# dominikbuenger/torch_nfft

Hardware: AMD Instinct MI355X
Metric: Mpoints/s (adjoint+forward, 3-D N=256 m=4) (higher is better)
Workload: dtype f32

## Files before the change

torch_nfft_amd/csrc/colfft.hip:

```cpp
#include <type_traits>

#include "common.h"
#include "kernels.h"

namespace nfft {

namespace {

constexpr int kFftThreads = 256;

struct ColGeom {
    int M, logM, N, H;
    int Mh;
    int SR;
    int KC;
    int KS;
    int NB;
    int NBm;
    int two_d;
    int NC, logNC;
    int TG;
    float param;
};

__device__ __forceinline__ float phi_hat_inv_f(int k, float param) { return expf((float)k * (float)k * param); }

__device__ __forceinline__ float2 cmul(float2 a, float2 b)
{
    return make_float2(a.x * b.x - a.y * b.y, a.x * b.y + a.y * b.x);
}

__device__ __forceinline__ void column_tile_of_block(const int tg, int &tile, int &row, int64_t &plane)
{
    const unsigned gx = gridDim.x, gy = gridDim.y;
    unsigned long long id = blockIdx.x + (unsigned long long)gx * (blockIdx.y + (unsigned long long)gy * blockIdx.z);
    if (tg > 1) {
        const unsigned long long total = (unsigned long long)gx * gy * gridDim.z;
        const unsigned span = 8u * (unsigned)tg;
        const unsigned long long base = id - id % span;
        if (base + span <= total) {
            const unsigned r = (unsigned)(id - base);
            id = base + (unsigned long long)(r & 7u) * (unsigned)tg + (r >> 3);
        }
    }
    tile = (int)(id % gx);
    const unsigned long long q = id / gx;
    row = (int)(q % gy);
    plane = (int64_t)(q / gy);
}

constexpr double kPiD = 3.14159265358979323846264338327950288;
constexpr double taylor_sin(double x)
{
    double term = x, sum = x;
    for (int k = 1; k <= 16; ++k) {
        term *= -x * x / (double)((2 * k) * (2 * k + 1));
        sum += term;
    }
    return sum;
}
constexpr double taylor_cos(double x)
{
    double term = 1.0, sum = 1.0;
    for (int k = 1; k <= 16; ++k) {
        term *= -x * x / (double)((2 * k - 1) * (2 * k));
        sum += term;
    }
    return sum;
}
struct TwPair { float x, y; };
template <int M>
struct TwTable { TwPair v[M / 2]; };
template <int M>
constexpr TwTable<M> make_tw_table()
{
    TwTable<M> t{};
    for (int j = 0; j < M / 2; ++j) {
        const bool upper = 4 * j > M;
        const double a = 2.0 * kPiD * (double)(upper ? M / 2 - j : j) / (double)M;
        const double c = taylor_cos(a), sn = taylor_sin(a);
        t.v[j] = TwPair{(float)(upper ? -c : c), (float)-sn};
    }
    return t;
}
template <int M>
__device__ const TwTable<M> kTwTable = make_tw_table<M>();

template <int M>
const float2 *tw_symbol()
{
    void *ptr = nullptr;
    if (hipGetSymbolAddress(&ptr, HIP_SYMBOL(kTwTable<M>)) != hipSuccess) return nullptr;
    return (const float2 *)ptr;
}
const float2 *twiddle_table(int M)
{
    static std::atomic<const float2 *> cache[kMaxDevices][7];
    const int dev = current_device();
    int slot = 0;
    while ((16 << slot) < M) ++slot;
    if (slot > 6 || (16 << slot) != M) return nullptr;
    if (dev < kMaxDevices) {
        const float2 *p = cache[dev][slot].load(std::memory_order_acquire);
        if (p) return p;
    }
    const float2 *p = nullptr;
    switch (M) {
    case 16: p = tw_symbol<16>(); break;
    case 32: p = tw_symbol<32>(); break;
    case 64: p = tw_symbol<64>(); break;
    case 128: p = tw_symbol<128>(); break;
    case 256: p = tw_symbol<256>(); break;
    case 512: p = tw_symbol<512>(); break;
    case 1024: p = tw_symbol<1024>(); break;
    }
    if (p && dev < kMaxDevices) cache[dev][slot].store(p, std::memory_order_release);
    return p;
}

__device__ __forceinline__ float2 cadd(float2 a, float2 b) { return make_float2(a.x + b.x, a.y + b.y); }
__device__ __forceinline__ float2 csub(float2 a, float2 b) { return make_float2(a.x - b.x, a.y - b.y); }
template <bool INV>
__device__ __forceinline__ float2 rot90(float2 a)
{
    return INV ? make_float2(-a.y, a.x) : make_float2(a.y, -a.x);
}

template <bool INV>
__device__ __forceinline__ void dft4(float2 &x0, float2 &x1, float2 &x2, float2 &x3)
{
    const float2 a0 = cadd(x0, x2), a1 = csub(x0, x2), a2 = cadd(x1, x3), a3 = rot90<INV>(csub(x1, x3));
    x0 = cadd(a0, a2);
    x1 = cadd(a1, a3);
    x2 = csub(a0, a2);
    x3 = csub(a1, a3);
}

template <bool INV>
__device__ __forceinline__ void dft8(float2 (&x)[8])
{
    dft4<INV>(x[0], x[2], x[4], x[6]);
    dft4<INV>(x[1], x[3], x[5], x[7]);
    constexpr float r = 0.70710678118654752440f;
    const float2 o0 = x[1];
    const float2 o1 = INV ? make_float2((x[3].x - x[3].y) * r, (x[3].x + x[3].y) * r)
                          : make_float2((x[3].x + x[3].y) * r, (x[3].y - x[3].x) * r);
    const float2 o2 = rot90<INV>(x[5]);
    const float2 o3 = INV ? make_float2((-x[7].x - x[7].y) * r, (x[7].x - x[7].y) * r)
                          : make_float2((x[7].y - x[7].x) * r, (-x[7].x - x[7].y) * r);
    const float2 e0 = x[0], e1 = x[2], e2 = x[4], e3 = x[6];
    x[0] = cadd(e0, o0); x[4] = csub(e0, o0);
    x[1] = cadd(e1, o1); x[5] = csub(e1, o1);
    x[2] = cadd(e2, o2); x[6] = csub(e2, o2);
    x[3] = cadd(e3, o3); x[7] = csub(e3, o3);
}

template <bool INV>
__device__ __forceinline__ float2 twiddle_at(const float2 *ltw, int e, int M)
{
    e &= M - 1;
    float2 w = ltw[e & (M / 2 - 1)];
    if (e >= M / 2) w = make_float2(-w.x, -w.y);
    if (INV) w.y = -w.y;
    return w;
}

template <bool INV, int R>
__device__ __forceinline__ void fft_stage(float2 *buf, const float2 *ltw, const ColGeom &cg, int tid, int logL)
{
    constexpr int logR = R == 8 ? 3 : 2;
    const int logLs = logL - logR, Ls = 1 << logLs;
    const int tstep = cg.M >> logL;
    const int total = (cg.M >> logR) << cg.logNC;
    __syncthreads();
    for (int idx = tid; idx < total; idx += kFftThreads) {
        const int col = idx & (cg.NC - 1);
        const int t = idx >> cg.logNC;
        const int j = t & (Ls - 1);
        const int row0 = ((t >> logLs) << logL) + j;
        float2 *p0 = buf + (row0 << cg.logNC) + col;
        const int stride = Ls << cg.logNC;
        float2 x[R];
#pragma unroll
        for (int q = 0; q < R; ++q) x[q] = p0[q * stride];
        if (R == 8) {
            dft8<INV>(reinterpret_cast<float2(&)[8]>(x));
        } else {
            dft4<INV>(x[0], x[1], x[2], x[3]);
        }
        p0[0] = x[0];
        if (logLs == 0) {
#pragma unroll
            for (int q = 1; q < R; ++q) p0[q * stride] = x[q];
        } else {
#pragma unroll
            for (int q = 1; q < R; ++q) p0[q * stride] = cmul(x[q], twiddle_at<INV>(ltw, j * q * tstep, cg.M));
        }
    }
}

template <bool INV>
__device__ __forceinline__ void lds_fft(float2 *buf, const float2 *ltw, const ColGeom &cg, int tid)
{
    switch (cg.logM) {
    case 4: fft_stage<INV, 4>(buf, ltw, cg, tid, 4); fft_stage<INV, 4>(buf, ltw, cg, tid, 2); break;
    case 5: fft_stage<INV, 8>(buf, ltw, cg, tid, 5); fft_stage<INV, 4>(buf, ltw, cg, tid, 2); break;
    case 6: fft_stage<INV, 8>(buf, ltw, cg, tid, 6); fft_stage<INV, 8>(buf, ltw, cg, tid, 3); break;
    case 7: fft_stage<INV, 8>(buf, ltw, cg, tid, 7); fft_stage<INV, 4>(buf, ltw, cg, tid, 4);
            fft_stage<INV, 4>(buf, ltw, cg, tid, 2); break;
    case 8: fft_stage<INV, 8>(buf, ltw, cg, tid, 8); fft_stage<INV, 8>(buf, ltw, cg, tid, 5);
            fft_stage<INV, 4>(buf, ltw, cg, tid, 2); break;
    case 9: fft_stage<INV, 8>(buf, ltw, cg, tid, 9); fft_stage<INV, 8>(buf, ltw, cg, tid, 6);
            fft_stage<INV, 8>(buf, ltw, cg, tid, 3); break;
    default: fft_stage<INV, 8>(buf, ltw, cg, tid, 10); fft_stage<INV, 8>(buf, ltw, cg, tid, 7);
             fft_stage<INV, 4>(buf, ltw, cg, tid, 4); fft_stage<INV, 4>(buf, ltw, cg, tid, 2); break;
    }
    __syncthreads();
}

__device__ __forceinline__ int brev_row(int k, int logM)
{
    int pos = 0, lg = logM;
    auto digit = [&](int lr) { lg -= lr; pos += (k & ((1 << lr) - 1)) << lg; k >>= lr; };
    switch (logM) {
    case 4: digit(2); digit(2); break;
    case 5: digit(3); digit(2); break;
    case 6: digit(3); digit(3); break;
    case 7: digit(3); digit(2); digit(2); break;
    case 8: digit(3); digit(3); digit(2); break;
    case 9: digit(3); digit(3); digit(3); break;
    default: digit(3); digit(3); digit(2); digit(2); break;
    }
    return pos;
}

template <int UN, typename LoadF, typename StoreF>
__device__ __forceinline__ void batched_fill(int total, int tid, LoadF load, StoreF store)
{
    for (int base = tid; base < total; base += kFftThreads * UN) {
        float2 v[UN];
#pragma unroll
        for (int r = 0; r < UN; ++r) {
            const int idx = base + r * kFftThreads;
            v[r] = idx < total ? load(idx) : make_float2(0.f, 0.f);
        }
#pragma unroll
        for (int r = 0; r < UN; ++r) {
            const int idx = base + r * kFftThreads;
            if (idx < total) store(idx, v[r]);
        }
    }
}

__device__ __forceinline__ void stage_twiddles(float2 *ltw, const float2 *__restrict__ tw, int M, int tid)
{
    for (int j = tid; j < M / 2; j += kFftThreads) ltw[j] = tw[j];
}

template <int LOGM, int LOGNC>
__global__ void __launch_bounds__(kFftThreads)
adj_axis1_kernel(ColGeom cg_in, const float2 *__restrict__ tw, const float2 *__restrict__ S, float2 *__restrict__ T)
{
    ColGeom cg = cg_in;
    if constexpr (LOGM > 0) {
        cg.M = 1 << LOGM;
        cg.logM = LOGM;
        cg.NC = 1 << LOGNC;
        cg.logNC = LOGNC;
    }
    extern __shared__ float2 smem[];
    float2 *ltw = smem;
    float2 *buf = smem + cg.M / 2;
    const int tid = threadIdx.x;
    int tile_x, u0;
    int64_t plane;
    column_tile_of_block(cg.TG, tile_x, u0, plane);
    const int c0 = tile_x << cg.logNC;
    if (c0 >= cg.KC) return;
    stage_twiddles(ltw, tw, cg.M, tid);
    const float2 *src = S + ((plane * cg.M + u0) * cg.M) * cg.SR;
    batched_fill<16>(cg.M << cg.logNC, tid,
                     [&](int idx) {
                         const int col = idx & (cg.NC - 1), u1 = idx >> cg.logNC;
                         const int k2 = c0 + col;
                         return k2 < cg.KC ? src[(int64_t)u1 * cg.SR + k2] : make_float2(0.f, 0.f);
                     },
                     [&](int idx, float2 v) { buf[idx] = v; });
    lds_fft<false>(buf, ltw, cg, tid);
    float2 *dst = T + ((plane * cg.M + u0) * cg.NB) * cg.KS;
    for (int idx = tid; idx < (cg.NB << cg.logNC); idx += kFftThreads) {
        const int col = idx & (cg.NC - 1), j1 = idx >> cg.logNC;
        const int k2 = c0 + col;
        if (k2 < cg.KC) {
            const int k1 = (j1 - cg.H) & (cg.M - 1);
            dst[(int64_t)j1 * cg.KS + k2] = buf[(brev_row(k1, cg.logM) << cg.logNC) + col];
        }
    }
}

__device__ __forceinline__ void apply_mult(const void *__restrict__ mult, int kind, int64_t f, float &re, float &im)
{
    if (kind == 1) {
        const float w = ((const float *)mult)[f];
        re *= w;
        im *= w;
    } else if (kind == 2) {
        const float2 w = ((const float2 *)mult)[f];
        const float r2 = re * w.x - im * w.y;
        im = re * w.y + im * w.x;
        re = r2;
    }
}

template <int LOGM, int LOGNC, bool XCOMPLEX, bool REAL_OUT>
__global__ void __launch_bounds__(kFftThreads)
adj_axis0_kernel(ColGeom cg_in, const float2 *__restrict__ tw, const float2 *__restrict__ T, int64_t C, int64_t col0,
                 void *__restrict__ yv, const void *__restrict__ mult, int mult_kind)
{
    ColGeom cg = cg_in;
    if constexpr (LOGM > 0) {
        cg.M = 1 << LOGM;
        cg.logM = LOGM;
        cg.NC = 1 << LOGNC;
        cg.logNC = LOGNC;
    }
    extern __shared__ float2 smem[];
    float2 *ltw = smem;
    float2 *buf = smem + cg.M / 2;
    float2 *buf2 = buf + (cg.M << cg.logNC);
    const int tid = threadIdx.x;
    int tile_x, j1;
    int64_t col_local;
    column_tile_of_block(cg.TG, tile_x, j1, col_local);
    const int c0 = tile_x << cg.logNC;
    if (c0 >= cg.KC) return;
    stage_twiddles(ltw, tw, cg.M, tid);
    const int64_t plane = XCOMPLEX ? col_local * 2 : col_local;
    const int64_t pstride = (int64_t)cg.M * cg.NBm * cg.KS;
    const float2 *src = T + plane * pstride + (int64_t)j1 * cg.KS;
    for (int part = 0; part < (XCOMPLEX ? 2 : 1); ++part) {
        float2 *const dstbuf = part ? buf2 : buf;
        const float2 *const srcp = src + part * pstride;
        batched_fill<16>(cg.M << cg.logNC, tid,
                         [&](int idx) {
                             const int col = idx & (cg.NC - 1), u0 = idx >> cg.logNC;
                             const int k2 = c0 + col;
                             return k2 < cg.KC ? srcp[(int64_t)u0 * cg.NBm * cg.KS + k2] : make_float2(0.f, 0.f);
                         },
                         [&](int idx, float2 v) { dstbuf[idx] = v; });
    }
    lds_fft<false>(buf, ltw, cg, tid);
    if (XCOMPLEX) lds_fft<false>(buf2, ltw, cg, tid);

    const int64_t colg = col0 + col_local;
    const int64_t b = colg / C, c = colg - b * C;
    const int H = cg.H, N = cg.N;
    const int k1 = cg.two_d ? 0 : j1 - H;
    const float f1 = cg.two_d ? 1.0f : phi_hat_inv_f(abs(k1), cg.param);
    const int64_t NN = cg.two_d ? (int64_t)N * N : (int64_t)N * N * N;
    for (int idx = tid; idx < (cg.NB << cg.logNC); idx += kFftThreads) {
        const int col = idx & (cg.NC - 1), j0 = idx >> cg.logNC;
        const int k2 = c0 + col;
        if (k2 >= cg.KC) continue;
        const int k0 = j0 - H;
        const int row = (brev_row(k0 & (cg.M - 1), cg.logM) << cg.logNC) + col;
        const float2 fr = buf[row];
        float2 fi = make_float2(0.f, 0.f);
        if (XCOMPLEX) fi = buf2[row];
        const float fac = phi_hat_inv_f(abs(k0), cg.param) * f1 * phi_hat_inv_f(k2, cg.param);
        if (k0 < H && k1 < H && k2 < H) {
            float re = (fr.x + fi.y) * fac, im = (-fr.y + fi.x) * fac;
            const int64_t f = cg.two_d ? (int64_t)(k0 + H) * N + (k2 + H) : ((int64_t)(k0 + H) * N + (k1 + H)) * N + (k2 + H);
            apply_mult(mult, mult_kind, f, re, im);
            const int64_t o = (b * NN + f) * C + c;
            if (REAL_OUT) ((float *)yv)[o] = re;
            else ((float2 *)yv)[o] = make_float2(re, im);
        }
        if (k2 >= 1 && k0 > -H && k1 > -H) {
            float re = (fr.x - fi.y) * fac, im = (fr.y + fi.x) * fac;
            const int64_t f = cg.two_d ? (int64_t)(H - k0) * N + (H - k2) : ((int64_t)(H - k0) * N + (H - k1)) * N + (H - k2);
            apply_mult(mult, mult_kind, f, re, im);
            const int64_t o = (b * NN + f) * C + c;
            if (REAL_OUT) ((float *)yv)[o] = re;
            else ((float2 *)yv)[o] = make_float2(re, im);
        }
    }
}

template <bool XCOMPLEX>
__device__ __forceinline__ float2 band_value(const void *__restrict__ xhat, int64_t b, int64_t c, int64_t C, int N,
                                             int H, int k0, int k1, int k2, const bool two_d = false)
{
    if (k0 < -H || k0 >= H || (!two_d && (k1 < -H || k1 >= H)) || k2 < -H || k2 >= H) return make_float2(0.f, 0.f);
    const int64_t idx = two_d ? ((b * N + (k0 + H)) * N + (k2 + H)) * C + c
                              : (((b * N + (k0 + H)) * N + (k1 + H)) * N + (k2 + H)) * C + c;
    if (XCOMPLEX) return ((const float2 *)xhat)[idx];
    return make_float2(((const float *)xhat)[idx], 0.f);
}

template <int LOGM, int LOGNC, bool XCOMPLEX>
__global__ void __launch_bounds__(kFftThreads)
fwd_axis0_kernel(ColGeom cg_in, const float2 *__restrict__ tw, const void *__restrict__ xhat, int64_t C, int ppc,
                 int64_t plane0, float2 *__restrict__ T)
{
    ColGeom cg = cg_in;
    if constexpr (LOGM > 0) {
        cg.M = 1 << LOGM;
        cg.logM = LOGM;
        cg.NC = 1 << LOGNC;
        cg.logNC = LOGNC;
    }
    extern __shared__ float2 smem[];
    float2 *ltw = smem;
    float2 *buf = smem + cg.M / 2;
    const int tid = threadIdx.x;
    int tile_x, j1;
    int64_t pl;
    column_tile_of_block(cg.TG, tile_x, j1, pl);
    const int c0 = tile_x << cg.logNC;
    if (c0 >= cg.KC) return;
    stage_twiddles(ltw, tw, cg.M, tid);
    for (int idx = tid; idx < (cg.M << cg.logNC); idx += kFftThreads) buf[idx] = make_float2(0.f, 0.f);
    __syncthreads();
    const int64_t plane = plane0 + pl;
    const int64_t colg = plane / ppc;
    const int part = (int)(plane - colg * ppc);
    const int64_t b = colg / C, c = colg - b * C;
    const int H = cg.H;
    const int k1 = cg.two_d ? 0 : j1 - H;
    const float f1 = cg.two_d ? 1.0f : phi_hat_inv_f(abs(k1), cg.param);
    batched_fill<8>(cg.NB << cg.logNC, tid,
                    [&](int idx) {
                        const int col = idx & (cg.NC - 1), j0 = idx >> cg.logNC;
                        const int k2 = c0 + col;
                        if (k2 >= cg.KC) return make_float2(0.f, 0.f);
                        const int k0 = j0 - H;
                        const float2 ap = band_value<XCOMPLEX>(xhat, b, c, C, cg.N, H, k0, k1, k2, cg.two_d != 0);
                        const float2 am = band_value<XCOMPLEX>(xhat, b, c, C, cg.N, H, -k0, -k1, -k2, cg.two_d != 0);
                        const float fac = 0.5f * phi_hat_inv_f(abs(k0), cg.param) * f1 * phi_hat_inv_f(k2, cg.param);
                        if (part == 0) return make_float2((am.x + ap.x) * fac, (am.y - ap.y) * fac);
                        return make_float2((am.y + ap.y) * fac, -(am.x - ap.x) * fac);
                    },
                    [&](int idx, float2 v) {
                        const int col = idx & (cg.NC - 1), j0 = idx >> cg.logNC;
                        if (c0 + col < cg.KC) buf[(((j0 - H) & (cg.M - 1)) << cg.logNC) + col] = v;
                    });
    lds_fft<true>(buf, ltw, cg, tid);
    float2 *dst = T + pl * ((int64_t)cg.M * cg.NBm * cg.KS) + (int64_t)j1 * cg.KS;
    for (int idx = tid; idx < (cg.M << cg.logNC); idx += kFftThreads) {
        const int col = idx & (cg.NC - 1), u0 = idx >> cg.logNC;
        const int k2 = c0 + col;
        if (k2 < cg.KC) dst[(int64_t)u0 * cg.NBm * cg.KS + k2] = buf[(brev_row(u0, cg.logM) << cg.logNC) + col];
    }
}

template <int LOGM, int LOGNC>
__global__ void __launch_bounds__(kFftThreads)
fwd_axis1_kernel(ColGeom cg_in, const float2 *__restrict__ tw, const float2 *__restrict__ T, float2 *__restrict__ S)
{
    ColGeom cg = cg_in;
    if constexpr (LOGM > 0) {
        cg.M = 1 << LOGM;
        cg.logM = LOGM;
        cg.NC = 1 << LOGNC;
        cg.logNC = LOGNC;
    }
    extern __shared__ float2 smem[];
    float2 *ltw = smem;
    float2 *buf = smem + cg.M / 2;
    const int tid = threadIdx.x;
    int tile_x, u0;
    int64_t plane;
    column_tile_of_block(cg.TG, tile_x, u0, plane);
    const int c0 = tile_x << cg.logNC;
    if (c0 >= (cg.SR == cg.KS ? cg.KC : cg.Mh)) return;
    float2 *dst = S + ((plane * cg.M + u0) * cg.M) * cg.SR;
    const int width = cg.SR == cg.KS ? cg.KC : cg.Mh;
    if (c0 >= cg.KC) {
        for (int idx = tid; idx < (cg.M << cg.logNC); idx += kFftThreads) {
            const int col = idx & (cg.NC - 1), u1 = idx >> cg.logNC;
            if (c0 + col < width) dst[(int64_t)u1 * cg.SR + c0 + col] = make_float2(0.f, 0.f);
        }
        return;
    }
    stage_twiddles(ltw, tw, cg.M, tid);
    for (int idx = tid; idx < (cg.M << cg.logNC); idx += kFftThreads) buf[idx] = make_float2(0.f, 0.f);
    __syncthreads();
    const float2 *src = T + ((plane * cg.M + u0) * cg.NB) * cg.KS;
    batched_fill<16>(cg.NB << cg.logNC, tid,
                     [&](int idx) {
                         const int col = idx & (cg.NC - 1), j1 = idx >> cg.logNC;
                         const int k2 = c0 + col;
                         return k2 < cg.KC ? src[(int64_t)j1 * cg.KS + k2] : make_float2(0.f, 0.f);
                     },
                     [&](int idx, float2 v) {
                         const int col = idx & (cg.NC - 1), j1 = idx >> cg.logNC;
                         if (c0 + col < cg.KC) buf[(((j1 - cg.H) & (cg.M - 1)) << cg.logNC) + col] = v;
                     });
    lds_fft<true>(buf, ltw, cg, tid);
    for (int idx = tid; idx < (cg.M << cg.logNC); idx += kFftThreads) {
        const int col = idx & (cg.NC - 1), u1 = idx >> cg.logNC;
        const int k2 = c0 + col;
        if (k2 < width) {
            dst[(int64_t)u1 * cg.SR + k2] =
                k2 < cg.KC ? buf[(brev_row(u1, cg.logM) << cg.logNC) + col] : make_float2(0.f, 0.f);
        }
    }
}

constexpr int kWaveCplx = 512;
constexpr int kRowWaves = 4;
constexpr int kR2cRounds = 1;
constexpr int kC2rRounds = 2;

__device__ __host__ constexpr int zsw(int i) { return i ^ ((i >> 3) & 0x1c) ^ ((i >> 2) & 3); }

template <bool INV, int R, int LOGLB, int LOGM>
__device__ __forceinline__ void wave_fft_stage(float2 *z, const float2 *ltw, int lane)
{
    constexpr int logR = R == 8 ? 3 : 2;
    constexpr int logLs = LOGLB - logR, Ls = 1 << logLs;
    constexpr int logT = LOGM - LOGLB;
    __builtin_amdgcn_wave_barrier();
#pragma unroll
    for (int t0 = 0; t0 < (kWaveCplx >> logR); t0 += 64) {
        const int t = t0 + lane;
        const int j = t & (Ls - 1);
        const int p0 = zsw(((t >> logLs) << LOGLB) + j);
        float2 x[R];
#pragma unroll
        for (int q = 0; q < R; ++q) x[q] = z[p0 ^ zsw(q * Ls)];
        if (R == 8) {
            dft8<INV>(reinterpret_cast<float2(&)[8]>(x));
        } else {
            dft4<INV>(x[0], x[1], x[2], x[3]);
        }
        z[p0] = x[0];
        if (logLs == 0) {
#pragma unroll
            for (int q = 1; q < R; ++q) z[p0 ^ zsw(q * Ls)] = x[q];
        } else {
            const int e1 = j << logT;
#pragma unroll
            for (int q = 1; q < R; ++q) {
                float2 w = ltw[(q * e1) & ((1 << LOGM) - 1)];
                if (INV) w.y = -w.y;
                z[p0 ^ zsw(q * Ls)] = cmul(x[q], w);
            }
        }
    }
    __builtin_amdgcn_wave_barrier();
}

template <bool INV, int LOGL>
__device__ __forceinline__ void wave_fft(float2 *z, const float2 *ltw, int lane)
{
    constexpr int LOGM = LOGL + 1;
    if constexpr (LOGL == 6) {
        wave_fft_stage<INV, 8, 6, LOGM>(z, ltw, lane); wave_fft_stage<INV, 8, 3, LOGM>(z, ltw, lane);
    } else if constexpr (LOGL == 7) {
        wave_fft_stage<INV, 8, 7, LOGM>(z, ltw, lane); wave_fft_stage<INV, 4, 4, LOGM>(z, ltw, lane);
        wave_fft_stage<INV, 4, 2, LOGM>(z, ltw, lane);
    } else if constexpr (LOGL == 8) {
        wave_fft_stage<INV, 8, 8, LOGM>(z, ltw, lane); wave_fft_stage<INV, 8, 5, LOGM>(z, ltw, lane);
        wave_fft_stage<INV, 4, 2, LOGM>(z, ltw, lane);
    } else {
        wave_fft_stage<INV, 8, 9, LOGM>(z, ltw, lane); wave_fft_stage<INV, 8, 6, LOGM>(z, ltw, lane);
        wave_fft_stage<INV, 8, 3, LOGM>(z, ltw, lane);
    }
}

template <int LOGL>
struct RowLds {
    float2 tw[2 << LOGL];
    float2 z[kRowWaves][kWaveCplx];
    unsigned short rev[1 << LOGL];
};

template <int LOGL>
__device__ __forceinline__ void row_tables(RowLds<LOGL> &S, const float2 *__restrict__ tw, int tid)
{
    constexpr int L = 1 << LOGL, M = 2 * L;
    for (int e = tid; e < M; e += kRowWaves * 64) {
        float2 w = tw[e & (L - 1)];
        if (e >= L) w = make_float2(-w.x, -w.y);
        S.tw[e] = w;
    }
    for (int k = tid; k < L; k += kRowWaves * 64) S.rev[k] = (unsigned short)brev_row(k, LOGL);
    __syncthreads();
}

template <int LOGL>
__global__ void __launch_bounds__(kRowWaves * 64)
row_r2c_kernel(int KC, int KS, int64_t nrows, const float2 *__restrict__ tw, const float *__restrict__ grid, float2 *__restrict__ out)
{
    constexpr int L = 1 << LOGL, M = 2 * L, RP = kWaveCplx / L;
    __shared__ RowLds<LOGL> S;
    const int tid = threadIdx.x, lane = tid & 63;
    const int wave = __builtin_amdgcn_readfirstlane(tid >> 6);
    float2 *z = S.z[wave];
    row_tables<LOGL>(S, tw, tid);
    const int64_t row0 = ((int64_t)blockIdx.x * kRowWaves + wave) * kR2cRounds * RP;
    float4 v4[kR2cRounds][kWaveCplx / 128];
#pragma unroll
    for (int r = 0; r < kR2cRounds; ++r) {
        const int64_t row = row0 + (int64_t)r * RP;
        const int nr = (int)max((int64_t)0, min((int64_t)RP, nrows - row));
        const float4 *src4 = (const float4 *)(grid + row * M);
#pragma unroll
        for (int q = 0; q < kWaveCplx / 128; ++q) {
            const int n2 = q * 64 + lane;
            v4[r][q] = 2 * n2 < nr * L ? src4[n2] : make_float4(0.f, 0.f, 0.f, 0.f);
        }
    }
#pragma unroll
    for (int r = 0; r < kR2cRounds; ++r) {
        const int64_t row = row0 + (int64_t)r * RP;
        if (row >= nrows) break;
        const int nr = (int)min((int64_t)RP, nrows - row);
#pragma unroll
        for (int q = 0; q < kWaveCplx / 128; ++q) {
            const int n2 = q * 64 + lane;
            z[zsw(2 * n2)] = make_float2(v4[r][q].x, v4[r][q].y);
            z[zsw(2 * n2 + 1)] = make_float2(v4[r][q].z, v4[r][q].w);
        }
        wave_fft<false, LOGL>(z, S.tw, lane);
        for (int rr = 0; rr < nr; ++rr) {
            float2 *dst = out + (row + rr) * KS;
            for (int k = lane; k < KC; k += 64) {
                const float2 a = z[zsw(rr * L + S.rev[k])];
                float2 b = z[zsw(rr * L + S.rev[(L - k) & (L - 1)])];
                b.y = -b.y;
                const float2 e = make_float2(0.5f * (a.x + b.x), 0.5f * (a.y + b.y));
                const float2 o = make_float2(0.5f * (a.x - b.x), 0.5f * (a.y - b.y));
                const float2 wo = cmul(S.tw[k], o);
                dst[k] = make_float2(e.x + wo.y, e.y - wo.x);
            }
        }
    }
}

template <int LOGL>
__global__ void __launch_bounds__(kRowWaves * 64)
row_c2r_kernel(int KC, int KS, int64_t nrows, const float2 *__restrict__ tw, const float2 *__restrict__ in, float *__restrict__ grid)
{
    constexpr int L = 1 << LOGL, M = 2 * L, RP = kWaveCplx / L;
    __shared__ RowLds<LOGL> S;
    const int tid = threadIdx.x, lane = tid & 63;
    const int wave = __builtin_amdgcn_readfirstlane(tid >> 6);
    float2 *z = S.z[wave];
    row_tables<LOGL>(S, tw, tid);
    const int64_t row0 = ((int64_t)blockIdx.x * kRowWaves + wave) * kC2rRounds * RP;
    constexpr int NIT = kWaveCplx / 64;
    float2 va[kC2rRounds][NIT];
#pragma unroll
    for (int r = 0; r < kC2rRounds; ++r) {
        const int64_t row = row0 + (int64_t)r * RP;
        const int nr = (int)max((int64_t)0, min((int64_t)RP, nrows - row));
        const float2 *src = in + row * KS;
#pragma unroll
        for (int it = 0; it < NIT; ++it) {
            const int n = it * 64 + lane;
            const int rr = n >> LOGL, k = n & (L - 1);
            const bool live = rr < nr;
            const int kk = k <= L / 2 ? k : L - k;
            va[r][it] = live ? src[rr * KS + kk] : make_float2(0.f, 0.f);
        }
    }
#pragma unroll
    for (int r = 0; r < kC2rRounds; ++r) {
        const int64_t row = row0 + (int64_t)r * RP;
        if (row >= nrows) break;
        const int nr = (int)min((int64_t)RP, nrows - row);
#pragma unroll
        for (int it = 0; it < NIT; ++it) {
            const int n = it * 64 + lane;
            const int k = n & (L - 1);
            const float2 v = va[r][it], zero = make_float2(0.f, 0.f);
            const float2 a = k <= L / 2 ? v : zero;
            float2 b = k >= L / 2 ? v : zero;
            b.y = -b.y;
            const float2 sum = make_float2(a.x + b.x, a.y + b.y), dif = make_float2(a.x - b.x, a.y - b.y);
            float2 w = S.tw[k];
            w.y = -w.y;
            const float2 wd = cmul(w, dif);
            z[zsw(n)] = make_float2(sum.x - wd.y, sum.y + wd.x);
        }
        wave_fft<true, LOGL>(z, S.tw, lane);
        float4 *dst4 = (float4 *)(grid + row * M);
#pragma unroll
        for (int q = 0; q < kWaveCplx / 128; ++q) {
            const int n2 = q * 64 + lane;
            const int na = 2 * n2, nb = 2 * n2 + 1;
            const int rr = na >> LOGL;
            if (rr < nr) {
                const float2 a = z[zsw(rr * L + S.rev[na & (L - 1)])], b = z[zsw(rr * L + S.rev[nb & (L - 1)])];
                dst4[n2] = make_float4(a.x, a.y, b.x, b.y);
            }
        }
    }
}

template <int LOGL>
__global__ void __launch_bounds__(kRowWaves * 64)
row_toeplitz_kernel(int KC, int KS, int64_t rows_per_plane, int64_t npairs, int64_t pair0, int64_t pairs_per_set,
                    const float2 *__restrict__ tw, const float *__restrict__ K, float2 *spec)
{
    constexpr int L = 1 << LOGL, M = 2 * L, RP = kWaveCplx / L, NIT = kWaveCplx / 64, NQ = kWaveCplx / 128;
    __shared__ RowLds<LOGL> S;
    const int tid = threadIdx.x, lane = tid & 63;
    const int wave = __builtin_amdgcn_readfirstlane(tid >> 6);
    float2 *z = S.z[wave];
    row_tables<LOGL>(S, tw, tid);
    const int64_t units_per_pair = rows_per_plane / RP;
    const int64_t unit = (int64_t)blockIdx.x * kRowWaves + wave;
    if (unit >= npairs * units_per_pair) return;
    const int64_t pair = unit / units_per_pair, rb = unit - pair * units_per_pair;
    const int64_t row_re = 2 * pair * rows_per_plane + rb * RP;
    const int64_t set = (pair0 + pair) / pairs_per_set;
    const float4 *k4 = (const float4 *)(K + (set * rows_per_plane + rb * RP) * M);
    float4 kv[NQ];
#pragma unroll
    for (int q = 0; q < NQ; ++q) kv[q] = k4[q * 64 + lane];
    float2 va[2][NIT];
#pragma unroll
    for (int pl = 0; pl < 2; ++pl) {
        const float2 *src = spec + (row_re + pl * rows_per_plane) * KS;
#pragma unroll
        for (int it = 0; it < NIT; ++it) {
            const int n = it * 64 + lane;
            const int rr = n >> LOGL, k = n & (L - 1);
            const int kk = k <= L / 2 ? k : L - k;
            va[pl][it] = src[rr * KS + kk];
        }
    }
#pragma unroll
    for (int pl = 0; pl < 2; ++pl) {
#pragma unroll
        for (int it = 0; it < NIT; ++it) {
            const int n = it * 64 + lane;
            const int k = n & (L - 1);
            const float2 v = va[pl][it], zero = make_float2(0.f, 0.f);
            const float2 a = k <= L / 2 ? v : zero;
            float2 b = k >= L / 2 ? v : zero;
            b.y = -b.y;
            const float2 sum = make_float2(a.x + b.x, a.y + b.y), dif = make_float2(a.x - b.x, a.y - b.y);
            float2 w = S.tw[k];
            w.y = -w.y;
            const float2 wd = cmul(w, dif);
            z[zsw(n)] = make_float2(sum.x - wd.y, sum.y + wd.x);
        }
        wave_fft<true, LOGL>(z, S.tw, lane);
        float4 v4[NQ];
#pragma unroll
        for (int q = 0; q < NQ; ++q) {
            const int n2 = q * 64 + lane;
            const int na = 2 * n2, nb = 2 * n2 + 1;
            const int rr = na >> LOGL;
            const float2 a = z[zsw(rr * L + S.rev[na & (L - 1)])], b = z[zsw(rr * L + S.rev[nb & (L - 1)])];
            v4[q] = make_float4(a.x * kv[q].x, a.y * kv[q].y, b.x * kv[q].z, b.y * kv[q].w);
        }
        __builtin_amdgcn_wave_barrier();
#pragma unroll
        for (int q = 0; q < NQ; ++q) {
            const int n2 = q * 64 + lane;
            z[zsw(2 * n2)] = make_float2(v4[q].x, v4[q].y);
            z[zsw(2 * n2 + 1)] = make_float2(v4[q].z, v4[q].w);
        }
        wave_fft<false, LOGL>(z, S.tw, lane);
        for (int rr = 0; rr < RP; ++rr) {
            float2 *dst = spec + (row_re + pl * rows_per_plane + rr) * KS;
            for (int k = lane; k < KC; k += 64) {
                const float2 a = z[zsw(rr * L + S.rev[k])];
                float2 b = z[zsw(rr * L + S.rev[(L - k) & (L - 1)])];
                b.y = -b.y;
                const float2 e = make_float2(0.5f * (a.x + b.x), 0.5f * (a.y + b.y));
                const float2 o = make_float2(0.5f * (a.x - b.x), 0.5f * (a.y - b.y));
                const float2 wo = cmul(S.tw[k], o);
                dst[k] = make_float2(e.x + wo.y, e.y - wo.x);
            }
        }
        __builtin_amdgcn_wave_barrier();
    }
}

constexpr int kCiQ = 16;
constexpr int kCiLogQ = 4;

template <int LOGL>
struct RowCiLds {
    float2 tw[2 << LOGL];
    float2 z[kCiQ][kWaveCplx];
    unsigned short rev[1 << LOGL];
};
__device__ __forceinline__ int xch_slot(int rk, int k2, int q) { return rk * kCiQ + (q ^ (k2 & (kCiQ - 1))); }

template <int LOGL>
__device__ __forceinline__ void row_ci_tables(RowCiLds<LOGL> &S, const float2 *__restrict__ tw, int tid)
{
    constexpr int L = 1 << LOGL, M = 2 * L;
    for (int e = tid; e < M; e += kCiQ * 64) {
        float2 w = tw[e & (L - 1)];
        if (e >= L) w = make_float2(-w.x, -w.y);
        S.tw[e] = w;
    }
    for (int k = tid; k < L; k += kCiQ * 64) S.rev[k] = (unsigned short)brev_row(k, LOGL);
    __syncthreads();
}

template <int LOGL>
__global__ void __launch_bounds__(kCiQ * 64)
row_r2c_ci_kernel(int64_t rows_per_plane, int64_t nplanes, const float2 *__restrict__ tw, const float *__restrict__ grid,
                  float2 *__restrict__ out)
{
    constexpr int L = 1 << LOGL, M = 2 * L, RP = kWaveCplx / L, KC = L / 2 + 1;
    extern __shared__ __align__(16) unsigned char smem_raw[];
    RowCiLds<LOGL> &S = *reinterpret_cast<RowCiLds<LOGL> *>(smem_raw);
    const int tid = threadIdx.x, lane = tid & 63;
    const int wave = __builtin_amdgcn_readfirstlane(tid >> 6);
    float2 *z = S.z[wave];
    row_ci_tables<LOGL>(S, tw, tid);
    const int64_t row0 = (int64_t)blockIdx.x * RP;
    const int64_t group = blockIdx.y;
    const int64_t plane = group * kCiQ + wave;
    const bool live = plane < nplanes;
    float4 v4[kWaveCplx / 128];
    const float4 *src4 = (const float4 *)(grid + (plane * rows_per_plane + row0) * M);
#pragma unroll
    for (int q = 0; q < kWaveCplx / 128; ++q) v4[q] = live ? src4[q * 64 + lane] : make_float4(0.f, 0.f, 0.f, 0.f);
#pragma unroll
    for (int q = 0; q < kWaveCplx / 128; ++q) {
        const int n2 = q * 64 + lane;
        z[zsw(2 * n2)] = make_float2(v4[q].x, v4[q].y);
        z[zsw(2 * n2 + 1)] = make_float2(v4[q].z, v4[q].w);
    }
    wave_fft<false, LOGL>(z, S.tw, lane);
    constexpr int NV = (RP * KC + 63) / 64;
    float2 vals[NV];
#pragma unroll
    for (int i = 0; i < NV; ++i) {
        const int t = i * 64 + lane;
        vals[i] = make_float2(0.f, 0.f);
        if (t < RP * KC) {
            const int rr = t / KC, k = t - rr * KC;
            const float2 a = z[zsw(rr * L + S.rev[k])];
            float2 b = z[zsw(rr * L + S.rev[(L - k) & (L - 1)])];
            b.y = -b.y;
            const float2 e = make_float2(0.5f * (a.x + b.x), 0.5f * (a.y + b.y));
            const float2 o = make_float2(0.5f * (a.x - b.x), 0.5f * (a.y - b.y));
            const float2 wo = cmul(S.tw[k], o);
            vals[i] = make_float2(e.x + wo.y, e.y - wo.x);
        }
    }
    __syncthreads();
    float2 *const xch = &S.z[0][0];
#pragma unroll
    for (int i = 0; i < NV; ++i) {
        const int t = i * 64 + lane;
        if (t < RP * KC) xch[xch_slot(t, t % KC, wave)] = vals[i];
    }
    __syncthreads();
    float2 *dst = out + ((group * rows_per_plane + row0) * KC) * kCiQ;
    for (int e = tid; e < RP * KC * kCiQ; e += kCiQ * 64) {
        const int rk = e >> kCiLogQ;
        dst[e] = xch[xch_slot(rk, rk % KC, e & (kCiQ - 1))];
    }
}

template <int LOGL>
__global__ void __launch_bounds__(kCiQ * 64)
row_c2r_ci_kernel(int64_t rows_per_plane, int64_t nplanes, const float2 *__restrict__ tw, const float2 *__restrict__ in,
                  float *__restrict__ grid)
{
    constexpr int L = 1 << LOGL, M = 2 * L, RP = kWaveCplx / L, KC = L / 2 + 1;
    extern __shared__ __align__(16) unsigned char smem_raw[];
    RowCiLds<LOGL> &S = *reinterpret_cast<RowCiLds<LOGL> *>(smem_raw);
    const int tid = threadIdx.x, lane = tid & 63;
    const int wave = __builtin_amdgcn_readfirstlane(tid >> 6);
    float2 *z = S.z[wave];
    const int64_t row0 = (int64_t)blockIdx.x * RP;
    const int64_t group = blockIdx.y;
    const int64_t plane = group * kCiQ + wave;
    const float2 *src = in + ((group * rows_per_plane + row0) * KC) * kCiQ;
    float2 *const xch = &S.z[0][0];
    for (int e = tid; e < RP * KC * kCiQ; e += kCiQ * 64) {
        const int rk = e >> kCiLogQ;
        xch[xch_slot(rk, rk % KC, e & (kCiQ - 1))] = src[e];
    }
    row_ci_tables<LOGL>(S, tw, tid);
    constexpr int NIT = kWaveCplx / 64;
    float2 va[NIT];
#pragma unroll
    for (int it = 0; it < NIT; ++it) {
        const int n = it * 64 + lane;
        const int rr = n >> LOGL, k = n & (L - 1);
        const int kk = k <= L / 2 ? k : L - k;
        va[it] = xch[xch_slot(rr * KC + kk, kk, wave)];
    }
    __syncthreads();
    if (plane >= nplanes) return;
#pragma unroll
    for (int it = 0; it < NIT; ++it) {
        const int n = it * 64 + lane;
        const int k = n & (L - 1);
        const float2 v = va[it], zero = make_float2(0.f, 0.f);
        const float2 a = k <= L / 2 ? v : zero;
        float2 b = k >= L / 2 ? v : zero;
        b.y = -b.y;
        const float2 sum = make_float2(a.x + b.x, a.y + b.y), dif = make_float2(a.x - b.x, a.y - b.y);
        float2 w = S.tw[k];
        w.y = -w.y;
        const float2 wd = cmul(w, dif);
        z[zsw(n)] = make_float2(sum.x - wd.y, sum.y + wd.x);
    }
    wave_fft<true, LOGL>(z, S.tw, lane);
    float4 *dst4 = (float4 *)(grid + (plane * rows_per_plane + row0) * M);
#pragma unroll
    for (int q = 0; q < kWaveCplx / 128; ++q) {
        const int n2 = q * 64 + lane;
        const int na = 2 * n2, nb = 2 * n2 + 1;
        const int rr = na >> LOGL;
        const float2 a = z[zsw(rr * L + S.rev[na & (L - 1)])], b = z[zsw(rr * L + S.rev[nb & (L - 1)])];
        dst4[n2] = make_float4(a.x, a.y, b.x, b.y);
    }
}

__global__ void __launch_bounds__(kFftThreads)
adj_axis1_ci_kernel(ColGeom cg, const float2 *__restrict__ tw, const float2 *__restrict__ S, float2 *__restrict__ T)
{
    extern __shared__ float2 smem[];
    float2 *ltw = smem;
    float2 *buf = smem + cg.M / 2;
    const int tid = threadIdx.x;
    const int k2 = blockIdx.x, u0 = blockIdx.y;
    const int64_t group = blockIdx.z;
    stage_twiddles(ltw, tw, cg.M, tid);
    const int64_t rs = (int64_t)cg.KC * kCiQ;
    const float2 *src = S + ((group * cg.M + u0) * cg.M) * rs + (int64_t)k2 * kCiQ;
    batched_fill<16>(cg.M << kCiLogQ, tid,
                     [&](int idx) { return src[(int64_t)(idx >> kCiLogQ) * rs + (idx & (kCiQ - 1))]; },
                     [&](int idx, float2 v) { buf[idx] = v; });
    lds_fft<false>(buf, ltw, cg, tid);
    float2 *dst = T + ((group * cg.M + u0) * cg.NB) * rs + (int64_t)k2 * kCiQ;
    for (int idx = tid; idx < (cg.NB << kCiLogQ); idx += kFftThreads) {
        const int q = idx & (kCiQ - 1), j1 = idx >> kCiLogQ;
        const int k1 = (j1 - cg.H) & (cg.M - 1);
        dst[(int64_t)j1 * rs + q] = buf[(brev_row(k1, cg.logM) << kCiLogQ) + q];
    }
}

template <bool XCOMPLEX, bool REAL_OUT>
__global__ void __launch_bounds__(kFftThreads)
adj_axis0_ci_kernel(ColGeom cg, const float2 *__restrict__ tw, const float2 *__restrict__ T, int64_t C, int64_t plane0,
                    int64_t nplanes, void *__restrict__ yv, const void *__restrict__ mult, int mult_kind)
{
    extern __shared__ float2 smem[];
    float2 *ltw = smem;
    float2 *buf = smem + cg.M / 2;
    const int tid = threadIdx.x;
    const int k2 = blockIdx.x, j1 = blockIdx.y;
    const int64_t group = blockIdx.z;
    stage_twiddles(ltw, tw, cg.M, tid);
    const int64_t rs = (int64_t)cg.KC * kCiQ;
    const float2 *src = T + (group * cg.M * cg.NB + j1) * rs + (int64_t)k2 * kCiQ;
    batched_fill<16>(cg.M << kCiLogQ, tid,
                     [&](int idx) { return src[(int64_t)(idx >> kCiLogQ) * cg.NB * rs + (idx & (kCiQ - 1))]; },
                     [&](int idx, float2 v) { buf[idx] = v; });
    lds_fft<false>(buf, ltw, cg, tid);

    const int H = cg.H, N = cg.N;
    const int k1 = j1 - H;
    const float f12 = phi_hat_inv_f(abs(k1), cg.param) * phi_hat_inv_f(k2, cg.param);
    constexpr int PPC = XCOMPLEX ? 2 : 1;
    for (int idx = tid; idx < (cg.NB << kCiLogQ); idx += kFftThreads) {
        const int q = idx & (kCiQ - 1), j0 = idx >> kCiLogQ;
        if (XCOMPLEX && (q & 1)) continue;
        const int64_t pl = group * kCiQ + q;
        if (pl >= nplanes) continue;
        const int64_t colg = (plane0 + pl) / PPC;
        const int64_t b = colg / C, c = colg - b * C;
        const int k0 = j0 - H;
        const int row = (brev_row(k0 & (cg.M - 1), cg.logM) << kCiLogQ) + q;
        const float2 fr = buf[row];
        float2 fi = make_float2(0.f, 0.f);
        if (XCOMPLEX) fi = buf[row + 1];
        const float fac = phi_hat_inv_f(abs(k0), cg.param) * f12;
        if (k0 < H && k1 < H && k2 < H) {
            float re = (fr.x + fi.y) * fac, im = (-fr.y + fi.x) * fac;
            const int64_t f = ((int64_t)(k0 + H) * N + (k1 + H)) * N + (k2 + H);
            apply_mult(mult, mult_kind, f, re, im);
            const int64_t o = (b * N * N * N + f) * C + c;
            if (REAL_OUT) ((float *)yv)[o] = re;
            else ((float2 *)yv)[o] = make_float2(re, im);
        }
        if (k2 >= 1 && k0 > -H && k1 > -H) {
            float re = (fr.x - fi.y) * fac, im = (fr.y + fi.x) * fac;
            const int64_t f = ((int64_t)(H - k0) * N + (H - k1)) * N + (H - k2);
            apply_mult(mult, mult_kind, f, re, im);
            const int64_t o = (b * N * N * N + f) * C + c;
            if (REAL_OUT) ((float *)yv)[o] = re;
            else ((float2 *)yv)[o] = make_float2(re, im);
        }
    }
}

template <bool XCOMPLEX>
__global__ void __launch_bounds__(kFftThreads)
fwd_axis0_ci_kernel(ColGeom cg, const float2 *__restrict__ tw, const void *__restrict__ xhat, int64_t C, int ppc,
                    int64_t plane0, int64_t nplanes, float2 *__restrict__ T)
{
    extern __shared__ float2 smem[];
    float2 *ltw = smem;
    float2 *buf = smem + cg.M / 2;
    const int tid = threadIdx.x;
    const int k2 = blockIdx.x, j1 = blockIdx.y;
    const int64_t group = blockIdx.z;
    stage_twiddles(ltw, tw, cg.M, tid);
    for (int idx = tid; idx < (cg.M << kCiLogQ); idx += kFftThreads) buf[idx] = make_float2(0.f, 0.f);
    __syncthreads();
    const int H = cg.H;
    const int k1 = j1 - H;
    const float f12 = 0.5f * phi_hat_inv_f(abs(k1), cg.param) * phi_hat_inv_f(k2, cg.param);
    batched_fill<8>(cg.NB << kCiLogQ, tid,
                    [&](int idx) {
                        const int q = idx & (kCiQ - 1), j0 = idx >> kCiLogQ;
                        const int64_t pl = group * kCiQ + q;
                        if (pl >= nplanes) return make_float2(0.f, 0.f);
                        const int64_t plane = plane0 + pl;
                        const int64_t colg = plane / ppc;
                        const int part = (int)(plane - colg * ppc);
                        const int64_t b = colg / C, c = colg - b * C;
                        const int k0 = j0 - H;
                        const float2 ap = band_value<XCOMPLEX>(xhat, b, c, C, cg.N, H, k0, k1, k2);
                        const float2 am = band_value<XCOMPLEX>(xhat, b, c, C, cg.N, H, -k0, -k1, -k2);
                        const float fac = phi_hat_inv_f(abs(k0), cg.param) * f12;
                        if (part == 0) return make_float2((am.x + ap.x) * fac, (am.y - ap.y) * fac);
                        return make_float2((am.y + ap.y) * fac, -(am.x - ap.x) * fac);
                    },
                    [&](int idx, float2 v) {
                        const int q = idx & (kCiQ - 1), j0 = idx >> kCiLogQ;
                        buf[(((j0 - H) & (cg.M - 1)) << kCiLogQ) + q] = v;
                    });
    lds_fft<true>(buf, ltw, cg, tid);
    const int64_t rs = (int64_t)cg.KC * kCiQ;
    float2 *dst = T + (group * cg.M * cg.NB + j1) * rs + (int64_t)k2 * kCiQ;
    for (int idx = tid; idx < (cg.M << kCiLogQ); idx += kFftThreads) {
        const int q = idx & (kCiQ - 1), u0 = idx >> kCiLogQ;
        dst[(int64_t)u0 * cg.NB * rs + q] = buf[(brev_row(u0, cg.logM) << kCiLogQ) + q];
    }
}

__global__ void __launch_bounds__(kFftThreads)
fwd_axis1_ci_kernel(ColGeom cg, const float2 *__restrict__ tw, const float2 *__restrict__ T, float2 *__restrict__ S)
{
    extern __shared__ float2 smem[];
    float2 *ltw = smem;
    float2 *buf = smem + cg.M / 2;
    const int tid = threadIdx.x;
    const int k2 = blockIdx.x, u0 = blockIdx.y;
    const int64_t group = blockIdx.z;
    stage_twiddles(ltw, tw, cg.M, tid);
    for (int idx = tid; idx < (cg.M << kCiLogQ); idx += kFftThreads) buf[idx] = make_float2(0.f, 0.f);
    __syncthreads();
    const int64_t rs = (int64_t)cg.KC * kCiQ;
    const float2 *src = T + ((group * cg.M + u0) * cg.NB) * rs + (int64_t)k2 * kCiQ;
    batched_fill<16>(cg.NB << kCiLogQ, tid,
                     [&](int idx) { return src[(int64_t)(idx >> kCiLogQ) * rs + (idx & (kCiQ - 1))]; },
                     [&](int idx, float2 v) {
                         const int q = idx & (kCiQ - 1), j1 = idx >> kCiLogQ;
                         buf[(((j1 - cg.H) & (cg.M - 1)) << kCiLogQ) + q] = v;
                     });
    lds_fft<true>(buf, ltw, cg, tid);
    float2 *dst = S + ((group * cg.M + u0) * cg.M) * rs + (int64_t)k2 * kCiQ;
    for (int idx = tid; idx < (cg.M << kCiLogQ); idx += kFftThreads) {
        const int q = idx & (kCiQ - 1), u1 = idx >> kCiLogQ;
        dst[(int64_t)u1 * rs + q] = buf[(brev_row(u1, cg.logM) << kCiLogQ) + q];
    }
}

template <typename T, bool TO_INTERLEAVED>
__global__ void __launch_bounds__(256)
column_layout_kernel(const T *__restrict__ src, T *__restrict__ dst, int64_t K , int64_t C, int64_t col0,
                     int64_t ncols)
{
    __shared__ T tile[32][65];
    const int64_t k0 = (int64_t)blockIdx.x * 64;
    const int64_t cl0 = (int64_t)blockIdx.y * 32;
    const int tid = threadIdx.x;
    if (TO_INTERLEAVED) {
        for (int e = tid; e < 32 * 64; e += 256) {
            const int cl = e >> 6, k = e & 63;
            if (cl0 + cl < ncols && k0 + k < K) tile[cl][k] = src[(cl0 + cl) * K + k0 + k];
        }
        __syncthreads();
        for (int e = tid; e < 32 * 64; e += 256) {
            const int k = e >> 5, cl = e & 31;
            if (cl0 + cl < ncols && k0 + k < K) {
                const int64_t colg = col0 + cl0 + cl, b = colg / C, c = colg - b * C;
                dst[(b * K + k0 + k) * C + c] = tile[cl][k];
            }
        }
    } else {
        for (int e = tid; e < 32 * 64; e += 256) {
            const int k = e >> 5, cl = e & 31;
            if (cl0 + cl < ncols && k0 + k < K) {
                const int64_t colg = col0 + cl0 + cl, b = colg / C, c = colg - b * C;
                tile[cl][k] = src[(b * K + k0 + k) * C + c];
            }
        }
        __syncthreads();
        for (int e = tid; e < 32 * 64; e += 256) {
            const int cl = e >> 6, k = e & 63;
            if (cl0 + cl < ncols && k0 + k < K) dst[(cl0 + cl) * K + k0 + k] = tile[cl][k];
        }
    }
}

int compact_stride(const Geom &g)
{
    const int a = g.M >= 512 ? 8 : 4;
    return (g.N / 2 + 1 + a - 1) / a * a;
}

ColGeom make_col_geom(const Geom &g, bool two_buffers, bool compact, int64_t planes = 0)
{
    ColGeom cg;
    cg.M = g.M;
    cg.logM = 0;
    while ((1 << cg.logM) < g.M) ++cg.logM;
    cg.N = g.N;
    cg.H = g.N / 2;
    cg.Mh = g.M / 2 + 1;
    cg.KC = cg.H + 1;
    cg.KS = compact_stride(g);
    cg.SR = compact ? cg.KS : cg.Mh;
    cg.NB = g.N + 1;
    cg.two_d = g.dim == 2;
    cg.NBm = cg.two_d ? 1 : cg.NB;
    int nc = 16;
    const int64_t cap = g.M >= 1024 ? 65536 : 32768;
    while (nc > 1 && (int64_t)g.M * nc * 8 * (two_buffers ? 2 : 1) > cap) nc >>= 1;
    if (g.dim == 2 && planes > 0)
        while (nc > 4 && ((g.N / 2 + 1 + nc - 1) / nc) * planes < 64) nc >>= 1;
    cg.NC = nc;
    cg.logNC = 0;
    while ((1 << cg.logNC) < nc) ++cg.logNC;
    cg.param = g.rolloff ? 1.047197551196597746f * (float)g.m / ((float)g.N * (float)g.N) : 0.0f;
    cg.TG = nc >= 16 ? 1 : 16 / nc;
    return cg;
}

static inline unsigned col_tiles(const ColGeom &cg, int columns = 0)
{
    const int t = ((columns > 0 ? columns : cg.KC) + cg.NC - 1) / cg.NC;
    return (unsigned)((t + cg.TG - 1) / cg.TG * cg.TG);
}

size_t col_lds_bytes(const ColGeom &cg, bool two_buffers)
{
    return (size_t)(cg.M / 2 + (int64_t)cg.M * cg.NC * (two_buffers ? 2 : 1)) * sizeof(float2);
}

template <typename K>
void allow_lds(K kernel, size_t bytes)
{
    if (bytes > 48 * 1024) (void)hipFuncSetAttribute((const void *)kernel, hipFuncAttributeMaxDynamicSharedMemorySize, (int)bytes);
}

}

bool colfft_supported(const Geom &g)
{
    if (g.dim == 2) return g.M >= 128 && g.M <= 1024 && (g.M & (g.M - 1)) == 0;
    return g.dim == 3 && g.M >= 16 && g.M <= 1024 && (g.M & (g.M - 1)) == 0;
}

int64_t colfft_scratch_bytes(const Geom &g, int64_t nplanes)
{
    return align_up(nplanes * (int64_t)g.M * (g.dim == 2 ? 1 : g.N + 1) * compact_stride(g) * 8, 256) + align_up((int64_t)g.M * 4, 256);
}

template <typename F>
static void col_dispatch(const ColGeom &cg, F &&f)
{
    using std::integral_constant;
    if (cg.logM == 9 && cg.logNC == 3) return f(integral_constant<int, 9>{}, integral_constant<int, 3>{});
    if (cg.logM == 9 && cg.logNC == 2) return f(integral_constant<int, 9>{}, integral_constant<int, 2>{});
    return f(integral_constant<int, 0>{}, integral_constant<int, 0>{});
}

int launch_colfft_adjoint(const Geom &g, const float2 *spec, bool compact, void *scratch, int64_t scratch_planes,
                          int64_t C, int x_is_complex, int real_output, int64_t plane0, int64_t nplanes, void *y,
                          const void *mult, int mult_kind, hipStream_t stream)
{
    if (nplanes <= 0) return 0;
    const float2 *T = (const float2 *)scratch;
    const float2 *tw = twiddle_table(g.M);
    if (!tw) { set_error("no twiddle table for this grid size"); return 4; }
    if (g.dim == 2) {
        if (!compact) { set_error("2-D column passes need the compact half spectrum of the own row passes"); return 4; }
        T = spec;
    } else {
        const ColGeom cg = make_col_geom(g, false, compact);
        const dim3 grid(col_tiles(cg), g.M, (unsigned)nplanes);
        const size_t lds = col_lds_bytes(cg, false);
        col_dispatch(cg, [&](auto lm, auto ln) {
            constexpr int LM = decltype(lm)::value, LN = decltype(ln)::value;
            allow_lds(adj_axis1_kernel<LM, LN>, lds);
            hipLaunchKernelGGL((adj_axis1_kernel<LM, LN>), grid, dim3(kFftThreads), lds, stream, cg, tw, spec, (float2 *)scratch);
        });
    }
    {
        const bool two = x_is_complex != 0;
        const int ppc = two ? 2 : 1;
        const int64_t col0 = plane0 / ppc, ncols = nplanes / ppc;
        const ColGeom cg = make_col_geom(g, two, compact, ncols);
        const dim3 grid(col_tiles(cg), cg.NBm, (unsigned)ncols);
        const size_t lds = col_lds_bytes(cg, two);
        col_dispatch(cg, [&](auto lm, auto ln) {
            constexpr int LM = decltype(lm)::value, LN = decltype(ln)::value;
            auto go = [&](auto kernel) {
                allow_lds(kernel, lds);
                hipLaunchKernelGGL(kernel, grid, dim3(kFftThreads), lds, stream, cg, tw, T, C, col0, y, mult, mult_kind);
            };
            if (two) {
                if (real_output) go(adj_axis0_kernel<LM, LN, true, true>);
                else go(adj_axis0_kernel<LM, LN, true, false>);
            } else {
                if (real_output) go(adj_axis0_kernel<LM, LN, false, true>);
                else go(adj_axis0_kernel<LM, LN, false, false>);
            }
        });
    }
    NFFT_HIP_CHECK(hipGetLastError());
    return 0;
}

int launch_colfft_forward(const Geom &g, const void *xhat, void *scratch, int64_t scratch_planes, int64_t C,
                          int x_is_complex, int real_output, int64_t plane0, int64_t nplanes, float2 *spec, bool compact,
                          hipStream_t stream)
{
    if (nplanes <= 0) return 0;
    float2 *T = (float2 *)scratch;
    const float2 *tw = twiddle_table(g.M);
    if (!tw) { set_error("no twiddle table for this grid size"); return 4; }
    if (g.dim == 2) {
        if (!compact) { set_error("2-D column passes need the compact half spectrum of the own row passes"); return 4; }
        T = spec;
    }
    const ColGeom cg = make_col_geom(g, false, compact, nplanes);
    const size_t lds = col_lds_bytes(cg, false);
    const int ppc = real_output ? 1 : 2;
    col_dispatch(cg, [&](auto lm, auto ln) {
        constexpr int LM = decltype(lm)::value, LN = decltype(ln)::value;
        {
            const dim3 grid(col_tiles(cg), cg.NBm, (unsigned)nplanes);
            if (x_is_complex) {
                allow_lds(fwd_axis0_kernel<LM, LN, true>, lds);
                hipLaunchKernelGGL((fwd_axis0_kernel<LM, LN, true>), grid, dim3(kFftThreads), lds, stream, cg, tw, xhat, C, ppc, plane0, T);
            } else {
                allow_lds(fwd_axis0_kernel<LM, LN, false>, lds);
                hipLaunchKernelGGL((fwd_axis0_kernel<LM, LN, false>), grid, dim3(kFftThreads), lds, stream, cg, tw, xhat, C, ppc, plane0, T);
            }
        }
        if (g.dim != 2) {
            const dim3 grid(col_tiles(cg, compact ? cg.KC : cg.Mh), g.M, (unsigned)nplanes);
            allow_lds(fwd_axis1_kernel<LM, LN>, lds);
            hipLaunchKernelGGL((fwd_axis1_kernel<LM, LN>), grid, dim3(kFftThreads), lds, stream, cg, tw, T, spec);
        }
    });
    NFFT_HIP_CHECK(hipGetLastError());
    return 0;
}

bool colfft_ci_supported(const Geom &g) { return g.dim == 3 && colfft_supported(g) && g.M >= 128 && g.M <= 1024; }

int64_t colfft_ci_planes(int64_t nplanes) { return (nplanes + kCiQ - 1) / kCiQ * kCiQ; }

static ColGeom make_ci_geom(const Geom &g)
{
    ColGeom cg = make_col_geom(g, false, true);
    cg.NC = kCiQ;
    cg.logNC = kCiLogQ;
    return cg;
}

template <int LOGL>
static int launch_rows_ci_t(bool c2r, const Geom &g, int64_t nplanes, const float2 *tw, const void *in, void *out,
                            hipStream_t stream)
{
    constexpr int RP = kWaveCplx >> LOGL;
    const int64_t rows = (int64_t)g.M * g.M;
    const dim3 blocks((unsigned)(rows / RP), (unsigned)((nplanes + kCiQ - 1) / kCiQ));
    const size_t lds = sizeof(RowCiLds<LOGL>);
    static DeviceOnce attr_done;
    if (attr_done.first_use()) {
        NFFT_HIP_CHECK(hipFuncSetAttribute((const void *)row_r2c_ci_kernel<LOGL>, hipFuncAttributeMaxDynamicSharedMemorySize, (int)lds));
        NFFT_HIP_CHECK(hipFuncSetAttribute((const void *)row_c2r_ci_kernel<LOGL>, hipFuncAttributeMaxDynamicSharedMemorySize, (int)lds));
        attr_done.mark();
    }
    if (c2r)
        hipLaunchKernelGGL((row_c2r_ci_kernel<LOGL>), blocks, dim3(kCiQ * 64), lds, stream, rows, nplanes, tw, (const float2 *)in,
                           (float *)out);
    else
        hipLaunchKernelGGL((row_r2c_ci_kernel<LOGL>), blocks, dim3(kCiQ * 64), lds, stream, rows, nplanes, tw, (const float *)in,
                           (float2 *)out);
    NFFT_HIP_CHECK(hipGetLastError());
    return 0;
}

static int launch_rows_ci(bool c2r, const Geom &g, int64_t nplanes, const void *in, void *out, hipStream_t stream)
{
    if (nplanes <= 0) return 0;
    const float2 *tw = twiddle_table(g.M);
    if (!tw) { set_error("no twiddle table for this grid size"); return 4; }
    switch (g.M) {
    case 128: return launch_rows_ci_t<6>(c2r, g, nplanes, tw, in, out, stream);
    case 256: return launch_rows_ci_t<7>(c2r, g, nplanes, tw, in, out, stream);
    case 512: return launch_rows_ci_t<8>(c2r, g, nplanes, tw, in, out, stream);
    case 1024: return launch_rows_ci_t<9>(c2r, g, nplanes, tw, in, out, stream);
    }
    set_error("row passes support M = 128 .. 1024");
    return 1;
}

int launch_row_r2c_ci(const Geom &g, const float *grid, int64_t nplanes, float2 *spec, hipStream_t stream)
{
    return launch_rows_ci(false, g, nplanes, grid, spec, stream);
}
int launch_row_c2r_ci(const Geom &g, const float2 *spec, int64_t nplanes, float *grid, hipStream_t stream)
{
    return launch_rows_ci(true, g, nplanes, spec, grid, stream);
}

int launch_colfft_adjoint_ci(const Geom &g, const float2 *spec, void *scratch, int64_t C, int x_is_complex,
                             int real_output, int64_t plane0, int64_t nplanes, void *y, const void *mult, int mult_kind,
                             hipStream_t stream)
{
    if (nplanes <= 0) return 0;
    float2 *T = (float2 *)scratch;
    const float2 *tw = twiddle_table(g.M);
    if (!tw) { set_error("no twiddle table for this grid size"); return 4; }
    const ColGeom cg = make_ci_geom(g);
    const size_t lds = col_lds_bytes(cg, false);
    const unsigned groups = (unsigned)((nplanes + kCiQ - 1) / kCiQ);
    allow_lds(adj_axis1_ci_kernel, lds);
    hipLaunchKernelGGL(adj_axis1_ci_kernel, dim3(cg.KC, g.M, groups), dim3(kFftThreads), lds, stream, cg, tw, spec, T);
    auto go = [&](auto kernel) {
        allow_lds(kernel, lds);
        hipLaunchKernelGGL(kernel, dim3(cg.KC, cg.NB, groups), dim3(kFftThreads), lds, stream, cg, tw, T, C, plane0, nplanes, y,
                           mult, mult_kind);
    };
    if (x_is_complex) {
        if (real_output) go(adj_axis0_ci_kernel<true, true>);
        else go(adj_axis0_ci_kernel<true, false>);
    } else {
        if (real_output) go(adj_axis0_ci_kernel<false, true>);
        else go(adj_axis0_ci_kernel<false, false>);
    }
    NFFT_HIP_CHECK(hipGetLastError());
    return 0;
}

int launch_colfft_forward_ci(const Geom &g, const void *xhat, float2 *spec, void *scratch, int64_t C, int x_is_complex,
                             int real_output, int64_t plane0, int64_t nplanes, hipStream_t stream)
{
    if (nplanes <= 0) return 0;
    float2 *T = (float2 *)scratch;
    const float2 *tw = twiddle_table(g.M);
    if (!tw) { set_error("no twiddle table for this grid size"); return 4; }
    const ColGeom cg = make_ci_geom(g);
    const size_t lds = col_lds_bytes(cg, false);
    const unsigned groups = (unsigned)((nplanes + kCiQ - 1) / kCiQ);
    const int ppc = real_output ? 1 : 2;
    if (x_is_complex) {
        allow_lds(fwd_axis0_ci_kernel<true>, lds);
        hipLaunchKernelGGL((fwd_axis0_ci_kernel<true>), dim3(cg.KC, cg.NB, groups), dim3(kFftThreads), lds, stream, cg, tw, xhat, C,
                           ppc, plane0, nplanes, T);
    } else {
        allow_lds(fwd_axis0_ci_kernel<false>, lds);
        hipLaunchKernelGGL((fwd_axis0_ci_kernel<false>), dim3(cg.KC, cg.NB, groups), dim3(kFftThreads), lds, stream, cg, tw, xhat, C,
                           ppc, plane0, nplanes, T);
    }
    allow_lds(fwd_axis1_ci_kernel, lds);
    hipLaunchKernelGGL(fwd_axis1_ci_kernel, dim3(cg.KC, g.M, groups), dim3(kFftThreads), lds, stream, cg, tw, T, spec);
    NFFT_HIP_CHECK(hipGetLastError());
    return 0;
}

bool rowfft_supported(const Geom &g)
{
    return colfft_supported(g) && g.M >= 128 && g.M <= 1024;
}

template <int LOGL>
static void launch_rows_t(bool c2r, const Geom &g, int64_t nrows, const float2 *tw, const void *in, void *out,
                          hipStream_t stream)
{
    const int64_t per_wg = (int64_t)kRowWaves * (c2r ? kC2rRounds : kR2cRounds) * (kWaveCplx >> LOGL);
    const dim3 blocks((unsigned)((nrows + per_wg - 1) / per_wg));
    if (c2r)
        hipLaunchKernelGGL((row_c2r_kernel<LOGL>), blocks, dim3(kRowWaves * 64), 0, stream, g.N / 2 + 1, compact_stride(g), nrows, tw,
                           (const float2 *)in, (float *)out);
    else
        hipLaunchKernelGGL((row_r2c_kernel<LOGL>), blocks, dim3(kRowWaves * 64), 0, stream, g.N / 2 + 1, compact_stride(g), nrows, tw,
                           (const float *)in, (float2 *)out);
}

static int launch_rows(bool c2r, const Geom &g, int64_t nplanes, const float2 *tw, const void *in, void *out,
                       hipStream_t stream)
{
    const int64_t nrows = nplanes * g.Ma[0] * g.Ma[1];
    switch (g.M) {
    case 128: launch_rows_t<6>(c2r, g, nrows, tw, in, out, stream); break;
    case 256: launch_rows_t<7>(c2r, g, nrows, tw, in, out, stream); break;
    case 512: launch_rows_t<8>(c2r, g, nrows, tw, in, out, stream); break;
    case 1024: launch_rows_t<9>(c2r, g, nrows, tw, in, out, stream); break;
    default: set_error("row passes support M = 128 .. 1024"); return 1;
    }
    NFFT_HIP_CHECK(hipGetLastError());
    return 0;
}

int launch_row_r2c(const Geom &g, const float *grid, void *scratch, int64_t scratch_planes, int64_t nplanes,
                   float2 *spec, hipStream_t stream)
{
    if (nplanes <= 0) return 0;
    const float2 *tw = twiddle_table(g.M);
    if (!tw) { set_error("no twiddle table for this grid size"); return 4; }
    return launch_rows(false, g, nplanes, tw, grid, spec, stream);
}

int launch_row_c2r(const Geom &g, const float2 *spec, void *scratch, int64_t scratch_planes, int64_t nplanes,
                   float *grid, hipStream_t stream)
{
    if (nplanes <= 0) return 0;
    const float2 *tw = twiddle_table(g.M);
    if (!tw) { set_error("no twiddle table for this grid size"); return 4; }
    return launch_rows(true, g, nplanes, tw, spec, grid, stream);
}

template <int LOGL>
static void launch_row_toeplitz_t(const Geom &g, const float2 *tw, float2 *spec, const float *K, int64_t pairs_per_set,
                                  int64_t pair0, int64_t npairs, hipStream_t stream)
{
    const int64_t rows_per_plane = (int64_t)g.Ma[0] * g.Ma[1];
    const int64_t units = npairs * (rows_per_plane / (kWaveCplx >> LOGL));
    const dim3 blocks((unsigned)((units + kRowWaves - 1) / kRowWaves));
    hipLaunchKernelGGL((row_toeplitz_kernel<LOGL>), blocks, dim3(kRowWaves * 64), 0, stream, g.N / 2 + 1, compact_stride(g),
                       rows_per_plane, npairs, pair0, pairs_per_set, tw, K, spec);
}

int launch_row_toeplitz(const Geom &g, float2 *spec, const float *K, int64_t pairs_per_set, int64_t pair0, int64_t npairs,
                        hipStream_t stream)
{
    if (npairs <= 0) return 0;
    const float2 *tw = twiddle_table(g.M);
    if (!tw) { set_error("no twiddle table for this grid size"); return 4; }
    switch (g.M) {
    case 128: launch_row_toeplitz_t<6>(g, tw, spec, K, pairs_per_set, pair0, npairs, stream); break;
    case 256: launch_row_toeplitz_t<7>(g, tw, spec, K, pairs_per_set, pair0, npairs, stream); break;
    case 512: launch_row_toeplitz_t<8>(g, tw, spec, K, pairs_per_set, pair0, npairs, stream); break;
    case 1024: launch_row_toeplitz_t<9>(g, tw, spec, K, pairs_per_set, pair0, npairs, stream); break;
    default: set_error("row passes support M = 128 .. 1024"); return 1;
    }
    NFFT_HIP_CHECK(hipGetLastError());
    return 0;
}

int launch_column_layout(bool to_interleaved, const void *src, void *dst, int64_t K, int64_t C, int64_t col0,
                         int64_t ncols, int elem_bytes, hipStream_t stream)
{
    if (ncols <= 0 || K <= 0) return 0;
    const dim3 blocks((unsigned)((K + 63) / 64), (unsigned)((ncols + 31) / 32));
    if (elem_bytes == 8) {
        if (to_interleaved)
            hipLaunchKernelGGL((column_layout_kernel<float2, true>), blocks, dim3(256), 0, stream, (const float2 *)src,
                               (float2 *)dst, K, C, col0, ncols);
        else
            hipLaunchKernelGGL((column_layout_kernel<float2, false>), blocks, dim3(256), 0, stream, (const float2 *)src,
                               (float2 *)dst, K, C, col0, ncols);
    } else {
        if (to_interleaved)
            hipLaunchKernelGGL((column_layout_kernel<float, true>), blocks, dim3(256), 0, stream, (const float *)src,
                               (float *)dst, K, C, col0, ncols);
        else
            hipLaunchKernelGGL((column_layout_kernel<float, false>), blocks, dim3(256), 0, stream, (const float *)src,
                               (float *)dst, K, C, col0, ncols);
    }
    NFFT_HIP_CHECK(hipGetLastError());
    return 0;
}

}
```

Measured before the change: 2789.

## Software-pipeline column FFT tiles with register prefetch and grouped multi-row blocks

Column-pass kernels now loop over a run of tiles and rows per workgroup. Each iteration issues the global loads for the next tile into registers before running the current tile's LDS FFT, and defers the current tile's output stores into the next iteration. It also adds optional 16-byte vectorized loads and stores and raises the launch-bounds occupancy hint. A compile-time mode mask picks paired, plain or grouped tiling and the wide accesses per pass, so the plain and grouped paths are enabled only for the forward passes. The goal is to overlap global memory latency with LDS compute and cut per-block setup cost, at the price of more registers and more complex control flow.

```diff
diff --git a/torch_nfft_amd/csrc/colfft.hip b/torch_nfft_amd/csrc/colfft.hip
--- a/torch_nfft_amd/csrc/colfft.hip
+++ b/torch_nfft_amd/csrc/colfft.hip
@@ -1,3 +1,4 @@
+#include <cstdint>
 #include <type_traits>
 
 #include "common.h"
@@ -8,6 +9,7 @@
 namespace {
 
 constexpr int kFftThreads = 256;
+constexpr int kColWavesPerSimd = 4;
 
 struct ColGeom {
     int M, logM, N, H;
@@ -20,6 +22,9 @@
     int two_d;
     int NC, logNC;
     int TG;
+    int RR;
+    int WIDE;
+    int GROUPED;
     float param;
 };
 
@@ -30,23 +35,41 @@
     return make_float2(a.x * b.x - a.y * b.y, a.x * b.y + a.y * b.x);
 }
 
-__device__ __forceinline__ void column_tile_of_block(const int tg, int &tile, int &row, int64_t &plane)
-{
+struct TileRun {
+    int tile, tile_end;
+    int row, row_end;
+    int64_t plane;
+};
+__device__ __forceinline__ TileRun tile_run_of_block(const ColGeom &cg, const int columns, const int rows)
+{
+    TileRun r;
+    const int tiles = (columns + cg.NC - 1) >> cg.logNC;
+    if (cg.GROUPED) {
+        r.tile = (int)blockIdx.x * cg.TG;
+        r.tile_end = min(r.tile + cg.TG, tiles);
+        r.row = (int)blockIdx.y * cg.RR;
+        r.row_end = min(r.row + cg.RR, rows);
+        r.plane = blockIdx.z;
+        return r;
+    }
     const unsigned gx = gridDim.x, gy = gridDim.y;
     unsigned long long id = blockIdx.x + (unsigned long long)gx * (blockIdx.y + (unsigned long long)gy * blockIdx.z);
-    if (tg > 1) {
+    if (cg.TG > 1) {
         const unsigned long long total = (unsigned long long)gx * gy * gridDim.z;
-        const unsigned span = 8u * (unsigned)tg;
+        const unsigned span = 8u * (unsigned)cg.TG;
         const unsigned long long base = id - id % span;
         if (base + span <= total) {
-            const unsigned r = (unsigned)(id - base);
-            id = base + (unsigned long long)(r & 7u) * (unsigned)tg + (r >> 3);
-        }
-    }
-    tile = (int)(id % gx);
+            const unsigned q = (unsigned)(id - base);
+            id = base + (unsigned long long)(q & 7u) * (unsigned)cg.TG + (q >> 3);
+        }
+    }
+    r.tile = (int)(id % gx);
+    r.tile_end = min(r.tile + 1, tiles);
     const unsigned long long q = id / gx;
-    row = (int)(q % gy);
-    plane = (int64_t)(q / gy);
+    r.row = (int)(q % gy);
+    r.row_end = r.row + 1;
+    r.plane = (int64_t)(q / gy);
+    return r;
 }
 
 constexpr double kPiD = 3.14159265358979323846264338327950288;
@@ -235,9 +258,9 @@
 }
 
 template <int UN, typename LoadF, typename StoreF>
-__device__ __forceinline__ void batched_fill(int total, int tid, LoadF load, StoreF store)
-{
-    for (int base = tid; base < total; base += kFftThreads * UN) {
+__device__ __forceinline__ void batched_fill(int total, int tid, LoadF load, StoreF store, int first = 0)
+{
+    for (int base = first + tid; base < total; base += kFftThreads * UN) {
         float2 v[UN];
 #pragma unroll
         for (int r = 0; r < UN; ++r) {
@@ -252,13 +275,87 @@
     }
 }
 
+constexpr int kTilePre = 16;
+
+__device__ __forceinline__ void tile_fence() { __builtin_amdgcn_sched_barrier(0); }
+
+__device__ __forceinline__ int tile_thread(int tid)
+{
+    asm volatile("" : "+v"(tid));
+    return tid;
+}
+
+template <int UN, typename AtF, typename LiveF>
+__device__ __forceinline__ void tile_request(float2 (&v)[UN], int total, int tid, bool wide, AtF at, LiveF live)
+{
+    static_assert(UN % 2 == 0, "two elements per 16-byte access");
+    if (wide) {
+#pragma unroll
+        for (int r = 0; r < UN / 2; ++r) {
+            const int idx = 2 * (tid + r * kFftThreads);
+            const float4 q = idx < total ? *(const float4 *)at(idx) : make_float4(0.f, 0.f, 0.f, 0.f);
+            v[2 * r] = make_float2(q.x, q.y);
+            v[2 * r + 1] = make_float2(q.z, q.w);
+        }
+    } else {
+#pragma unroll
+        for (int r = 0; r < UN; ++r) {
+            const int idx = tid + r * kFftThreads;
+            v[r] = idx < total && live(idx) ? *at(idx) : make_float2(0.f, 0.f);
+        }
+    }
+}
+
+template <int UN, typename AtF, typename LiveF, typename PosF, typename KeepF>
+__device__ __forceinline__ void tile_commit(const float2 (&v)[UN], float2 *buf, int total, int tid, bool wide, AtF at, LiveF live,
+                                            PosF pos, KeepF keep)
+{
+    if (wide) {
+#pragma unroll
+        for (int r = 0; r < UN / 2; ++r) {
+            const int idx = 2 * (tid + r * kFftThreads);
+            if (idx < total) *(float4 *)(buf + pos(idx)) = make_float4(v[2 * r].x, v[2 * r].y, v[2 * r + 1].x, v[2 * r + 1].y);
+        }
+    } else {
+#pragma unroll
+        for (int r = 0; r < UN; ++r) {
+            const int idx = tid + r * kFftThreads;
+            if (idx < total && keep(idx)) buf[pos(idx)] = v[r];
+        }
+    }
+    batched_fill<16>(total, tid, [&](int idx) { return live(idx) ? *at(idx) : make_float2(0.f, 0.f); },
+                     [&](int idx, float2 w) { if (keep(idx)) buf[pos(idx)] = w; }, UN * kFftThreads);
+}
+
+template <int UN, typename FromF>
+__device__ __forceinline__ void tile_take(float2 (&o)[UN], const float2 *buf, int npairs, int tid, FromF from)
+{
+#pragma unroll
+    for (int r = 0; r < UN / 2; ++r) {
+        const int p = tid + r * kFftThreads;
+        const float4 q = p < npairs ? *(const float4 *)(buf + from(p)) : make_float4(0.f, 0.f, 0.f, 0.f);
+        o[2 * r] = make_float2(q.x, q.y);
+        o[2 * r + 1] = make_float2(q.z, q.w);
+    }
+}
+
+template <int UN, typename ToF>
+__device__ __forceinline__ void tile_send(const float2 (&o)[UN], int npairs, int tid, ToF to)
+{
+#pragma unroll
+    for (int r = 0; r < UN / 2; ++r) {
+        const int p = tid + r * kFftThreads;
+        if (p < npairs) *(float4 *)to(p) = make_float4(o[2 * r].x, o[2 * r].y, o[2 * r + 1].x, o[2 * r + 1].y);
+    }
+}
+
 __device__ __forceinline__ void stage_twiddles(float2 *ltw, const float2 *__restrict__ tw, int M, int tid)
 {
     for (int j = tid; j < M / 2; j += kFftThreads) ltw[j] = tw[j];
 }
 
 template <int LOGM, int LOGNC>
-__global__ void __launch_bounds__(kFftThreads)
+__global__ void __launch_bounds__(kFftThreads, kColWavesPerSimd)
 adj_axis1_kernel(ColGeom cg_in, const float2 *__restrict__ tw, const float2 *__restrict__ S, float2 *__restrict__ T)
 {
     ColGeom cg = cg_in;
@@ -268,34 +365,82 @@
         cg.NC = 1 << LOGNC;
         cg.logNC = LOGNC;
     }
-    extern __shared__ float2 smem[];
+    extern __shared__ __align__(16) float2 smem[];
     float2 *ltw = smem;
     float2 *buf = smem + cg.M / 2;
-    const int tid = threadIdx.x;
-    int tile_x, u0;
-    int64_t plane;
-    column_tile_of_block(cg.TG, tile_x, u0, plane);
-    const int c0 = tile_x << cg.logNC;
-    if (c0 >= cg.KC) return;
+    const int tid = threadIdx.x, tid0 = tid;
+    const TileRun run = tile_run_of_block(cg, cg.KC, cg.M);
+    if (run.tile >= run.tile_end) return;
+    const int64_t plane = run.plane;
     stage_twiddles(ltw, tw, cg.M, tid);
-    const float2 *src = S + ((plane * cg.M + u0) * cg.M) * cg.SR;
-    batched_fill<16>(cg.M << cg.logNC, tid,
-                     [&](int idx) {
-                         const int col = idx & (cg.NC - 1), u1 = idx >> cg.logNC;
-                         const int k2 = c0 + col;
-                         return k2 < cg.KC ? src[(int64_t)u1 * cg.SR + k2] : make_float2(0.f, 0.f);
-                     },
-                     [&](int idx, float2 v) { buf[idx] = v; });
-    lds_fft<false>(buf, ltw, cg, tid);
-    float2 *dst = T + ((plane * cg.M + u0) * cg.NB) * cg.KS;
-    for (int idx = tid; idx < (cg.NB << cg.logNC); idx += kFftThreads) {
-        const int col = idx & (cg.NC - 1), j1 = idx >> cg.logNC;
-        const int k2 = c0 + col;
-        if (k2 < cg.KC) {
-            const int k1 = (j1 - cg.H) & (cg.M - 1);
-            dst[(int64_t)j1 * cg.KS + k2] = buf[(brev_row(k1, cg.logM) << cg.logNC) + col];
-        }
-    }
+    const int total = cg.M << cg.logNC;
+    const bool wide_in = cg.WIDE && cg.NC >= 2 && !(cg.SR & 1) && !((uintptr_t)S & 15);
+    const bool wide_out = cg.WIDE && cg.NC >= 2 && !((uintptr_t)T & 15);
+    auto whole = [&](int c0) { return c0 + cg.NC <= cg.KC; };
+    auto src_of = [&](int u0, int c0) { return S + ((plane * cg.M + u0) * cg.M) * cg.SR + c0; };
+    auto at_of = [&](const float2 *src) {
+        return [&cg, src](int idx) { return src + (int64_t)(idx >> cg.logNC) * cg.SR + (idx & (cg.NC - 1)); };
+    };
+    auto live_of = [&](int c0) { return [&cg, c0](int idx) { return c0 + (idx & (cg.NC - 1)) < cg.KC; }; };
+    float2 pre[kTilePre];
+    constexpr int kOut = 10;
+    const int opairs = cg.NB << (cg.logNC - 1);
+    const bool late_out = wide_out && opairs <= kFftThreads * (kOut / 2);
+    float2 out[kOut];
+    float2 *out_dst = nullptr;
+    auto send = [&](int tid) {
+        tile_send(out, opairs, tid, [&](int p) { return out_dst + (int64_t)(p >> (cg.logNC - 1)) * cg.KS + ((p << 1) & (cg.NC - 1)); });
+    };
+    int u0 = run.row, tile = run.tile;
+    tile_request(pre, total, tid, wide_in && whole(tile << cg.logNC), at_of(src_of(u0, tile << cg.logNC)), live_of(tile << cg.logNC));
+    while (true) {
+        const int tid = tile_thread(tid0);
+        const int c0 = tile << cg.logNC;
+        tile_commit(pre, buf, total, tid, wide_in && whole(c0), at_of(src_of(u0, c0)), live_of(c0), [](int idx) { return idx; },
+                    [](int) { return true; });
+        if (out_dst) send(tid);
+        out_dst = nullptr;
+        int u0n = u0, tilen = tile + 1;
+        if (tilen == run.tile_end) {
+            tilen = run.tile;
+            ++u0n;
+        }
+        const bool more = u0n < run.row_end;
+        tile_fence();
+        if (more) {
+            const int c0n = tilen << cg.logNC;
+            tile_request(pre, total, tid, wide_in && whole(c0n), at_of(src_of(u0n, c0n)), live_of(c0n));
+        }
+        tile_fence();
+        lds_fft<false>(buf, ltw, cg, tid);
+        float2 *dst = T + ((plane * cg.M + u0) * cg.NB) * cg.KS + c0;
+        if (late_out && whole(c0)) {
+            tile_take(out, buf, opairs, tid, [&](int p) {
+                const int k1 = ((p >> (cg.logNC - 1)) - cg.H) & (cg.M - 1);
+                return (brev_row(k1, cg.logM) << cg.logNC) + ((p << 1) & (cg.NC - 1));
+            });
+            out_dst = dst;
+        } else if (wide_out && whole(c0)) {
+            for (int p = tid; p < (cg.NB << (cg.logNC - 1)); p += kFftThreads) {
+                const int col = (p << 1) & (cg.NC - 1), j1 = p >> (cg.logNC - 1);
+                const int k1 = (j1 - cg.H) & (cg.M - 1);
+                *(float4 *)(dst + (int64_t)j1 * cg.KS + col) = *(const float4 *)(buf + (brev_row(k1, cg.logM) << cg.logNC) + col);
+            }
+        } else {
+            for (int idx = tid; idx < (cg.NB << cg.logNC); idx += kFftThreads) {
+                const int col = idx & (cg.NC - 1), j1 = idx >> cg.logNC;
+                if (c0 + col < cg.KC) {
+                    const int k1 = (j1 - cg.H) & (cg.M - 1);
+                    dst[(int64_t)j1 * cg.KS + col] = buf[(brev_row(k1, cg.logM) << cg.logNC) + col];
+                }
+            }
+        }
+        if (!more) break;
+        __syncthreads();
+        u0 = u0n;
+        tile = tilen;
+    }
+    if (out_dst) send(tid);
 }
 
 __device__ __forceinline__ void apply_mult(const void *__restrict__ mult, int kind, int64_t f, float &re, float &im)
@@ -312,52 +457,14 @@
     }
 }
 
-template <int LOGM, int LOGNC, bool XCOMPLEX, bool REAL_OUT>
-__global__ void __launch_bounds__(kFftThreads)
-adj_axis0_kernel(ColGeom cg_in, const float2 *__restrict__ tw, const float2 *__restrict__ T, int64_t C, int64_t col0,
-                 void *__restrict__ yv, const void *__restrict__ mult, int mult_kind)
-{
-    ColGeom cg = cg_in;
-    if constexpr (LOGM > 0) {
-        cg.M = 1 << LOGM;
-        cg.logM = LOGM;
-        cg.NC = 1 << LOGNC;
-        cg.logNC = LOGNC;
-    }
-    extern __shared__ float2 smem[];
-    float2 *ltw = smem;
-    float2 *buf = smem + cg.M / 2;
-    float2 *buf2 = buf + (cg.M << cg.logNC);
-    const int tid = threadIdx.x;
-    int tile_x, j1;
-    int64_t col_local;
-    column_tile_of_block(cg.TG, tile_x, j1, col_local);
-    const int c0 = tile_x << cg.logNC;
-    if (c0 >= cg.KC) return;
-    stage_twiddles(ltw, tw, cg.M, tid);
-    const int64_t plane = XCOMPLEX ? col_local * 2 : col_local;
-    const int64_t pstride = (int64_t)cg.M * cg.NBm * cg.KS;
-    const float2 *src = T + plane * pstride + (int64_t)j1 * cg.KS;
-    for (int part = 0; part < (XCOMPLEX ? 2 : 1); ++part) {
-        float2 *const dstbuf = part ? buf2 : buf;
-        const float2 *const srcp = src + part * pstride;
-        batched_fill<16>(cg.M << cg.logNC, tid,
-                         [&](int idx) {
-                             const int col = idx & (cg.NC - 1), u0 = idx >> cg.logNC;
-                             const int k2 = c0 + col;
-                             return k2 < cg.KC ? srcp[(int64_t)u0 * cg.NBm * cg.KS + k2] : make_float2(0.f, 0.f);
-                         },
-                         [&](int idx, float2 v) { dstbuf[idx] = v; });
-    }
-    lds_fft<false>(buf, ltw, cg, tid);
-    if (XCOMPLEX) lds_fft<false>(buf2, ltw, cg, tid);
-
-    const int64_t colg = col0 + col_local;
-    const int64_t b = colg / C, c = colg - b * C;
+template <bool XCOMPLEX, bool REAL_OUT>
+__device__ __forceinline__ void adj_axis0_store(const ColGeom &cg, const float2 *buf, const float2 *buf2, int tid, int c0, int j1,
+                                                int64_t b, int64_t c, int64_t C, int64_t NN, void *__restrict__ yv,
+                                                const void *__restrict__ mult, int mult_kind)
+{
     const int H = cg.H, N = cg.N;
     const int k1 = cg.two_d ? 0 : j1 - H;
     const float f1 = cg.two_d ? 1.0f : phi_hat_inv_f(abs(k1), cg.param);
-    const int64_t NN = cg.two_d ? (int64_t)N * N : (int64_t)N * N * N;
     for (int idx = tid; idx < (cg.NB << cg.logNC); idx += kFftThreads) {
         const int col = idx & (cg.NC - 1), j0 = idx >> cg.logNC;
         const int k2 = c0 + col;
@@ -387,21 +494,10 @@
     }
 }
 
-template <bool XCOMPLEX>
-__device__ __forceinline__ float2 band_value(const void *__restrict__ xhat, int64_t b, int64_t c, int64_t C, int N,
-                                             int H, int k0, int k1, int k2, const bool two_d = false)
-{
-    if (k0 < -H || k0 >= H || (!two_d && (k1 < -H || k1 >= H)) || k2 < -H || k2 >= H) return make_float2(0.f, 0.f);
-    const int64_t idx = two_d ? ((b * N + (k0 + H)) * N + (k2 + H)) * C + c
-                              : (((b * N + (k0 + H)) * N + (k1 + H)) * N + (k2 + H)) * C + c;
-    if (XCOMPLEX) return ((const float2 *)xhat)[idx];
-    return make_float2(((const float *)xhat)[idx], 0.f);
-}
-
-template <int LOGM, int LOGNC, bool XCOMPLEX>
-__global__ void __launch_bounds__(kFftThreads)
-fwd_axis0_kernel(ColGeom cg_in, const float2 *__restrict__ tw, const void *__restrict__ xhat, int64_t C, int ppc,
-                 int64_t plane0, float2 *__restrict__ T)
+template <int LOGM, int LOGNC, bool XCOMPLEX, bool REAL_OUT>
+__global__ void __launch_bounds__(kFftThreads, kColWavesPerSimd)
+adj_axis0_kernel(ColGeom cg_in, const float2 *__restrict__ tw, const float2 *__restrict__ T, int64_t C, int64_t col0,
+                 void *__restrict__ yv, const void *__restrict__ mult, int mult_kind)
 {
     ColGeom cg = cg_in;
     if constexpr (LOGM > 0) {
@@ -410,53 +506,83 @@
         cg.NC = 1 << LOGNC;
         cg.logNC = LOGNC;
     }
-    extern __shared__ float2 smem[];
+    extern __shared__ __align__(16) float2 smem[];
     float2 *ltw = smem;
     float2 *buf = smem + cg.M / 2;
-    const int tid = threadIdx.x;
-    int tile_x, j1;
-    int64_t pl;
-    column_tile_of_block(cg.TG, tile_x, j1, pl);
-    const int c0 = tile_x << cg.logNC;
-    if (c0 >= cg.KC) return;
+    float2 *buf2 = buf + (cg.M << cg.logNC);
+    const int tid = threadIdx.x, tid0 = tid;
+    const TileRun run = tile_run_of_block(cg, cg.KC, cg.NBm);
+    if (run.tile >= run.tile_end) return;
+    const int64_t col_local = run.plane;
     stage_twiddles(ltw, tw, cg.M, tid);
-    for (int idx = tid; idx < (cg.M << cg.logNC); idx += kFftThreads) buf[idx] = make_float2(0.f, 0.f);
-    __syncthreads();
-    const int64_t plane = plane0 + pl;
-    const int64_t colg = plane / ppc;
-    const int part = (int)(plane - colg * ppc);
+    const int64_t plane = XCOMPLEX ? col_local * 2 : col_local;
+    const int64_t pstride = (int64_t)cg.M * cg.NBm * cg.KS;
+    const int total = cg.M << cg.logNC;
+    const bool wide_in = cg.WIDE && cg.NC >= 2 && !((uintptr_t)T & 15);
+    auto whole = [&](int c0) { return c0 + cg.NC <= cg.KC; };
+    auto src_of = [&](int j1, int c0, int part) { return T + (plane + part) * pstride + (int64_t)j1 * cg.KS + c0; };
+    auto at_of = [&](const float2 *src) {
+        return [&cg, src](int idx) { return src + (int64_t)(idx >> cg.logNC) * cg.NBm * cg.KS + (idx & (cg.NC - 1)); };
+    };
+    auto live_of = [&](int c0) { return [&cg, c0](int idx) { return c0 + (idx & (cg.NC - 1)) < cg.KC; }; };
+    constexpr int NP = XCOMPLEX ? 2 : 1;
+    float2 pre[NP][kTilePre / NP];
+    int j1 = run.row, tile = run.tile;
+#pragma unroll
+    for (int part = 0; part < NP; ++part)
+        tile_request(pre[part], total, tid, wide_in && whole(tile << cg.logNC), at_of(src_of(j1, tile << cg.logNC, part)),
+                     live_of(tile << cg.logNC));
+    const int64_t colg = col0 + col_local;
     const int64_t b = colg / C, c = colg - b * C;
-    const int H = cg.H;
-    const int k1 = cg.two_d ? 0 : j1 - H;
-    const float f1 = cg.two_d ? 1.0f : phi_hat_inv_f(abs(k1), cg.param);
-    batched_fill<8>(cg.NB << cg.logNC, tid,
-                    [&](int idx) {
-                        const int col = idx & (cg.NC - 1), j0 = idx >> cg.logNC;
-                        const int k2 = c0 + col;
-                        if (k2 >= cg.KC) return make_float2(0.f, 0.f);
-                        const int k0 = j0 - H;
-                        const float2 ap = band_value<XCOMPLEX>(xhat, b, c, C, cg.N, H, k0, k1, k2, cg.two_d != 0);
-                        const float2 am = band_value<XCOMPLEX>(xhat, b, c, C, cg.N, H, -k0, -k1, -k2, cg.two_d != 0);
-                        const float fac = 0.5f * phi_hat_inv_f(abs(k0), cg.param) * f1 * phi_hat_inv_f(k2, cg.param);
-                        if (part == 0) return make_float2((am.x + ap.x) * fac, (am.y - ap.y) * fac);
-                        return make_float2((am.y + ap.y) * fac, -(am.x - ap.x) * fac);
-                    },
-                    [&](int idx, float2 v) {
-                        const int col = idx & (cg.NC - 1), j0 = idx >> cg.logNC;
-                        if (c0 + col < cg.KC) buf[(((j0 - H) & (cg.M - 1)) << cg.logNC) + col] = v;
-                    });
-    lds_fft<true>(buf, ltw, cg, tid);
-    float2 *dst = T + pl * ((int64_t)cg.M * cg.NBm * cg.KS) + (int64_t)j1 * cg.KS;
-    for (int idx = tid; idx < (cg.M << cg.logNC); idx += kFftThreads) {
-        const int col = idx & (cg.NC - 1), u0 = idx >> cg.logNC;
-        const int k2 = c0 + col;
-        if (k2 < cg.KC) dst[(int64_t)u0 * cg.NBm * cg.KS + k2] = buf[(brev_row(u0, cg.logM) << cg.logNC) + col];
-    }
-}
-
-template <int LOGM, int LOGNC>
-__global__ void __launch_bounds__(kFftThreads)
-fwd_axis1_kernel(ColGeom cg_in, const float2 *__restrict__ tw, const float2 *__restrict__ T, float2 *__restrict__ S)
+    const int64_t NN = cg.two_d ? (int64_t)cg.N * cg.N : (int64_t)cg.N * cg.N * cg.N;
+    while (true) {
+        const int tid = tile_thread(tid0);
+        const int c0 = tile << cg.logNC;
+#pragma unroll
+        for (int part = 0; part < NP; ++part)
+            tile_commit(pre[part], part ? buf2 : buf, total, tid, wide_in && whole(c0), at_of(src_of(j1, c0, part)), live_of(c0),
+                        [](int idx) { return idx; }, [](int) { return true; });
+        int j1n = j1, tilen = tile + 1;
+        if (tilen == run.tile_end) {
+            tilen = run.tile;
+            ++j1n;
+        }
+        const bool more = j1n < run.row_end;
+        tile_fence();
+        if (more) {
+            const int c0n = tilen << cg.logNC;
+#pragma unroll
+            for (int part = 0; part < NP; ++part)
+                tile_request(pre[part], total, tid, wide_in && whole(c0n), at_of(src_of(j1n, c0n, part)), live_of(c0n));
+        }
+        tile_fence();
+        lds_fft<false>(buf, ltw, cg, tid);
+        if (XCOMPLEX) lds_fft<false>(buf2, ltw, cg, tid);
+        adj_axis0_store<XCOMPLEX, REAL_OUT>(cg, buf, buf2, tid, c0, j1, b, c, C, NN, yv, mult, mult_kind);
+        if (!more) break;
+        __syncthreads();
+        j1 = j1n;
+        tile = tilen;
+    }
+}
+
+template <bool XCOMPLEX>
+__device__ __forceinline__ float2 band_value(const void *__restrict__ xhat, int64_t b, int64_t c, int64_t C, int N,
+                                             int H, int k0, int k1, int k2, const bool two_d = false)
+{
+    if (k0 < -H || k0 >= H || (!two_d && (k1 < -H || k1 >= H)) || k2 < -H || k2 >= H) return make_float2(0.f, 0.f);
+    const int64_t idx = two_d ? ((b * N + (k0 + H)) * N + (k2 + H)) * C + c
+                              : (((b * N + (k0 + H)) * N + (k1 + H)) * N + (k2 + H)) * C + c;
+    if (XCOMPLEX) return ((const float2 *)xhat)[idx];
+    return make_float2(((const float *)xhat)[idx], 0.f);
+}
+
+constexpr int kBandPre = 9;
+
+template <int LOGM, int LOGNC, bool XCOMPLEX>
+__global__ void __launch_bounds__(kFftThreads, kColWavesPerSimd)
+fwd_axis0_kernel(ColGeom cg_in, const float2 *__restrict__ tw, const void *__restrict__ xhat, int64_t C, int ppc,
+                 int64_t plane0, float2 *__restrict__ T)
 {
     ColGeom cg = cg_in;
     if constexpr (LOGM > 0) {
@@ -465,47 +591,214 @@
         cg.NC = 1 << LOGNC;
         cg.logNC = LOGNC;
     }
-    extern __shared__ float2 smem[];
+    extern __shared__ __align__(16) float2 smem[];
     float2 *ltw = smem;
     float2 *buf = smem + cg.M / 2;
-    const int tid = threadIdx.x;
-    int tile_x, u0;
-    int64_t plane;
-    column_tile_of_block(cg.TG, tile_x, u0, plane);
-    const int c0 = tile_x << cg.logNC;
-    if (c0 >= (cg.SR == cg.KS ? cg.KC : cg.Mh)) return;
-    float2 *dst = S + ((plane * cg.M + u0) * cg.M) * cg.SR;
+    const int tid = threadIdx.x, tid0 = tid;
+    const TileRun run = tile_run_of_block(cg, cg.KC, cg.NBm);
+    if (run.tile >= run.tile_end) return;
+    const int64_t pl = run.plane;
+    stage_twiddles(ltw, tw, cg.M, tid);
+    const int64_t plane = plane0 + pl;
+    const int64_t colg = plane / ppc;
+    const int part = (int)(plane - colg * ppc);
+    const int64_t b = colg / C, c = colg - b * C;
+    const int H = cg.H;
+    const int band = cg.NB << cg.logNC;
+    const bool wide_out = cg.WIDE && cg.NC >= 2 && !((uintptr_t)T & 15);
+    auto raw = [&](int idx, int j1, int c0, float2 &ap, float2 &am) {
+        const int col = idx & (cg.NC - 1), j0 = idx >> cg.logNC;
+        const int k2 = c0 + col;
+        ap = am = make_float2(0.f, 0.f);
+        if (k2 >= cg.KC) return;
+        const int k0 = j0 - H, k1 = cg.two_d ? 0 : j1 - H;
+        ap = band_value<XCOMPLEX>(xhat, b, c, C, cg.N, H, k0, k1, k2, cg.two_d != 0);
+        am = band_value<XCOMPLEX>(xhat, b, c, C, cg.N, H, -k0, -k1, -k2, cg.two_d != 0);
+    };
+    auto value = [&](int idx, int c0, float f1, float2 ap, float2 am) {
+        const int col = idx & (cg.NC - 1), j0 = idx >> cg.logNC;
+        const int k2 = c0 + col;
+        if (k2 >= cg.KC) return make_float2(0.f, 0.f);
+        const int k0 = j0 - H;
+        const float fac = 0.5f * phi_hat_inv_f(abs(k0), cg.param) * f1 * phi_hat_inv_f(k2, cg.param);
+        if (part == 0) return make_float2((am.x + ap.x) * fac, (am.y - ap.y) * fac);
+        return make_float2((am.y + ap.y) * fac, -(am.x - ap.x) * fac);
+    };
+    auto put = [&](int idx, int c0, float2 v) {
+        const int col = idx & (cg.NC - 1), j0 = idx >> cg.logNC;
+        if (c0 + col < cg.KC) buf[(((j0 - H) & (cg.M - 1)) << cg.logNC) + col] = v;
+    };
+    float2 pre_p[kBandPre], pre_m[kBandPre];
+    const int opairs = cg.M << (cg.logNC - 1);
+    const bool late_out = wide_out && opairs <= kFftThreads * (kTilePre / 2);
+    float2 out[kTilePre];
+    float2 *out_dst = nullptr;
+    auto send = [&](int tid) {
+        tile_send(out, opairs, tid,
+                  [&](int p) { return out_dst + (int64_t)(p >> (cg.logNC - 1)) * cg.NBm * cg.KS + ((p << 1) & (cg.NC - 1)); });
+    };
+    auto request = [&](int tid, int j1, int c0) {
+#pragma unroll
+        for (int r = 0; r < kBandPre; ++r) {
+            const int idx = tid + r * kFftThreads;
+            pre_p[r] = pre_m[r] = make_float2(0.f, 0.f);
+            if (idx < band) raw(idx, j1, c0, pre_p[r], pre_m[r]);
+        }
+    };
+    int j1 = run.row, tile = run.tile;
+    request(tid, j1, tile << cg.logNC);
+    while (true) {
+        const int tid = tile_thread(tid0);
+        const int c0 = tile << cg.logNC;
+        for (int idx = tid; idx < (cg.M << cg.logNC); idx += kFftThreads) buf[idx] = make_float2(0.f, 0.f);
+        __syncthreads();
+        const float f1 = cg.two_d ? 1.0f : phi_hat_inv_f(abs(j1 - H), cg.param);
+#pragma unroll
+        for (int r = 0; r < kBandPre; ++r) {
+            const int idx = tid + r * kFftThreads;
+            if (idx < band) put(idx, c0, value(idx, c0, f1, pre_p[r], pre_m[r]));
+        }
+        batched_fill<8>(band, tid,
+                        [&](int idx) {
+                            float2 ap, am;
+                            raw(idx, j1, c0, ap, am);
+                            return value(idx, c0, f1, ap, am);
+                        },
+                        [&](int idx, float2 v) { put(idx, c0, v); }, kBandPre * kFftThreads);
+        if (out_dst) send(tid);
+        out_dst = nullptr;
+        int j1n = j1, tilen = tile + 1;
+        if (tilen == run.tile_end) {
+            tilen = run.tile;
+            ++j1n;
+        }
+        const bool more = j1n < run.row_end;
+        tile_fence();
+        if (more) request(tid, j1n, tilen << cg.logNC);
+        tile_fence();
+        lds_fft<true>(buf, ltw, cg, tid);
+        float2 *dst = T + pl * ((int64_t)cg.M * cg.NBm * cg.KS) + (int64_t)j1 * cg.KS + c0;
+        if (late_out && c0 + cg.NC <= cg.KC) {
+            tile_take(out, buf, opairs, tid,
+                      [&](int p) { return (brev_row(p >> (cg.logNC - 1), cg.logM) << cg.logNC) + ((p << 1) & (cg.NC - 1)); });
+            out_dst = dst;
+        } else if (wide_out && c0 + cg.NC <= cg.KC) {
+            for (int p = tid; p < (cg.M << (cg.logNC - 1)); p += kFftThreads) {
+                const int col = (p << 1) & (cg.NC - 1), u0 = p >> (cg.logNC - 1);
+                *(float4 *)(dst + (int64_t)u0 * cg.NBm * cg.KS + col) = *(const float4 *)(buf + (brev_row(u0, cg.logM) << cg.logNC) + col);
+            }
+        } else {
+            for (int idx = tid; idx < (cg.M << cg.logNC); idx += kFftThreads) {
+                const int col = idx & (cg.NC - 1), u0 = idx >> cg.logNC;
+                if (c0 + col < cg.KC) dst[(int64_t)u0 * cg.NBm * cg.KS + col] = buf[(brev_row(u0, cg.logM) << cg.logNC) + col];
+            }
+        }
+        if (!more) break;
+        __syncthreads();
+        j1 = j1n;
+        tile = tilen;
+    }
+    if (out_dst) send(tid);
+}
+
+template <int LOGM, int LOGNC>
+__global__ void __launch_bounds__(kFftThreads, kColWavesPerSimd)
+fwd_axis1_kernel(ColGeom cg_in, const float2 *__restrict__ tw, const float2 *__restrict__ T, float2 *__restrict__ S)
+{
+    ColGeom cg = cg_in;
+    if constexpr (LOGM > 0) {
+        cg.M = 1 << LOGM;
+        cg.logM = LOGM;
+        cg.NC = 1 << LOGNC;
+        cg.logNC = LOGNC;
+    }
+    extern __shared__ __align__(16) float2 smem[];
+    float2 *ltw = smem;
+    float2 *buf = smem + cg.M / 2;
+    const int tid = threadIdx.x, tid0 = tid;
     const int width = cg.SR == cg.KS ? cg.KC : cg.Mh;
-    if (c0 >= cg.KC) {
-        for (int idx = tid; idx < (cg.M << cg.logNC); idx += kFftThreads) {
-            const int col = idx & (cg.NC - 1), u1 = idx >> cg.logNC;
-            if (c0 + col < width) dst[(int64_t)u1 * cg.SR + c0 + col] = make_float2(0.f, 0.f);
-        }
-        return;
-    }
+    const TileRun run = tile_run_of_block(cg, width, cg.M);
+    if (run.tile >= run.tile_end) return;
+    const int64_t plane = run.plane;
     stage_twiddles(ltw, tw, cg.M, tid);
-    for (int idx = tid; idx < (cg.M << cg.logNC); idx += kFftThreads) buf[idx] = make_float2(0.f, 0.f);
-    __syncthreads();
-    const float2 *src = T + ((plane * cg.M + u0) * cg.NB) * cg.KS;
-    batched_fill<16>(cg.NB << cg.logNC, tid,
-                     [&](int idx) {
-                         const int col = idx & (cg.NC - 1), j1 = idx >> cg.logNC;
-                         const int k2 = c0 + col;
-                         return k2 < cg.KC ? src[(int64_t)j1 * cg.KS + k2] : make_float2(0.f, 0.f);
-                     },
-                     [&](int idx, float2 v) {
-                         const int col = idx & (cg.NC - 1), j1 = idx >> cg.logNC;
-                         if (c0 + col < cg.KC) buf[(((j1 - cg.H) & (cg.M - 1)) << cg.logNC) + col] = v;
-                     });
-    lds_fft<true>(buf, ltw, cg, tid);
-    for (int idx = tid; idx < (cg.M << cg.logNC); idx += kFftThreads) {
-        const int col = idx & (cg.NC - 1), u1 = idx >> cg.logNC;
-        const int k2 = c0 + col;
-        if (k2 < width) {
-            dst[(int64_t)u1 * cg.SR + k2] =
-                k2 < cg.KC ? buf[(brev_row(u1, cg.logM) << cg.logNC) + col] : make_float2(0.f, 0.f);
-        }
-    }
+    const int band = cg.NB << cg.logNC;
+    const bool wide_in = cg.WIDE && cg.NC >= 2 && !((uintptr_t)T & 15);
+    const bool wide_out = cg.WIDE && cg.NC >= 2 && !(cg.SR & 1) && !((uintptr_t)S & 15);
+    auto whole = [&](int c0) { return c0 + cg.NC <= cg.KC; };
+    auto src_of = [&](int u0, int c0) { return T + ((plane * cg.M + u0) * cg.NB) * cg.KS + c0; };
+    auto at_of = [&](const float2 *src) {
+        return [&cg, src](int idx) { return src + (int64_t)(idx >> cg.logNC) * cg.KS + (idx & (cg.NC - 1)); };
+    };
+    auto live_of = [&](int c0) { return [&cg, c0](int idx) { return c0 + (idx & (cg.NC - 1)) < cg.KC; }; };
+    auto pos = [&cg](int idx) { return ((((idx >> cg.logNC) - cg.H) & (cg.M - 1)) << cg.logNC) + (idx & (cg.NC - 1)); };
+    float2 pre[kTilePre];
+    const int opairs = cg.M << (cg.logNC - 1);
+    const bool late_out = wide_out && opairs <= kFftThreads * (kTilePre / 2);
+    float2 out[kTilePre];
+    float2 *out_dst = nullptr;
+    auto send = [&](int tid) {
+        tile_send(out, opairs, tid, [&](int p) { return out_dst + (int64_t)(p >> (cg.logNC - 1)) * cg.SR + ((p << 1) & (cg.NC - 1)); });
+    };
+    int u0 = run.row, tile = run.tile;
+    if ((tile << cg.logNC) < cg.KC)
+        tile_request(pre, band, tid, wide_in && whole(tile << cg.logNC), at_of(src_of(u0, tile << cg.logNC)), live_of(tile << cg.logNC));
+    while (true) {
+        const int tid = tile_thread(tid0);
+        const int c0 = tile << cg.logNC;
+        const bool tail = c0 >= cg.KC;
+        if (!tail) {
+            for (int idx = tid; idx < (cg.M << cg.logNC); idx += kFftThreads) buf[idx] = make_float2(0.f, 0.f);
+            __syncthreads();
+            tile_commit(pre, buf, band, tid, wide_in && whole(c0), at_of(src_of(u0, c0)), live_of(c0), pos, live_of(c0));
+        }
+        if (out_dst) send(tid);
+        out_dst = nullptr;
+        int u0n = u0, tilen = tile + 1;
+        if (tilen == run.tile_end) {
+            tilen = run.tile;
+            ++u0n;
+        }
+        const bool more = u0n < run.row_end;
+        tile_fence();
+        if (more && (tilen << cg.logNC) < cg.KC) {
+            const int c0n = tilen << cg.logNC;
+            tile_request(pre, band, tid, wide_in && whole(c0n), at_of(src_of(u0n, c0n)), live_of(c0n));
+        }
+        tile_fence();
+        float2 *dst = S + ((plane * cg.M + u0) * cg.M) * cg.SR + c0;
+        if (tail) {
+            for (int idx = tid; idx < (cg.M << cg.logNC); idx += kFftThreads) {
+                const int col = idx & (cg.NC - 1), u1 = idx >> cg.logNC;
+                if (c0 + col < width) dst[(int64_t)u1 * cg.SR + col] = make_float2(0.f, 0.f);
+            }
+        } else {
+            lds_fft<true>(buf, ltw, cg, tid);
+            if (late_out && whole(c0)) {
+                tile_take(out, buf, opairs, tid,
+                          [&](int p) { return (brev_row(p >> (cg.logNC - 1), cg.logM) << cg.logNC) + ((p << 1) & (cg.NC - 1)); });
+                out_dst = dst;
+            } else if (wide_out && whole(c0)) {
+                for (int p = tid; p < (cg.M << (cg.logNC - 1)); p += kFftThreads) {
+                    const int col = (p << 1) & (cg.NC - 1), u1 = p >> (cg.logNC - 1);
+                    *(float4 *)(dst + (int64_t)u1 * cg.SR + col) = *(const float4 *)(buf + (brev_row(u1, cg.logM) << cg.logNC) + col);
+                }
+            } else {
+                for (int idx = tid; idx < (cg.M << cg.logNC); idx += kFftThreads) {
+                    const int col = idx & (cg.NC - 1), u1 = idx >> cg.logNC;
+                    const int k2 = c0 + col;
+                    if (k2 < width) {
+                        dst[(int64_t)u1 * cg.SR + col] =
+                            k2 < cg.KC ? buf[(brev_row(u1, cg.logM) << cg.logNC) + col] : make_float2(0.f, 0.f);
+                    }
+                }
+            }
+        }
+        if (!more) break;
+        __syncthreads();
+        u0 = u0n;
+        tile = tilen;
+    }
+    if (out_dst) send(tid);
 }
 
 constexpr int kWaveCplx = 512;
@@ -928,7 +1221,7 @@
 __global__ void __launch_bounds__(kFftThreads)
 adj_axis1_ci_kernel(ColGeom cg, const float2 *__restrict__ tw, const float2 *__restrict__ S, float2 *__restrict__ T)
 {
-    extern __shared__ float2 smem[];
+    extern __shared__ __align__(16) float2 smem[];
     float2 *ltw = smem;
     float2 *buf = smem + cg.M / 2;
     const int tid = threadIdx.x;
@@ -954,7 +1247,7 @@
 adj_axis0_ci_kernel(ColGeom cg, const float2 *__restrict__ tw, const float2 *__restrict__ T, int64_t C, int64_t plane0,
                     int64_t nplanes, void *__restrict__ yv, const void *__restrict__ mult, int mult_kind)
 {
-    extern __shared__ float2 smem[];
+    extern __shared__ __align__(16) float2 smem[];
     float2 *ltw = smem;
     float2 *buf = smem + cg.M / 2;
     const int tid = threadIdx.x;
@@ -1009,7 +1302,7 @@
 fwd_axis0_ci_kernel(ColGeom cg, const float2 *__restrict__ tw, const void *__restrict__ xhat, int64_t C, int ppc,
                     int64_t plane0, int64_t nplanes, float2 *__restrict__ T)
 {
-    extern __shared__ float2 smem[];
+    extern __shared__ __align__(16) float2 smem[];
     float2 *ltw = smem;
     float2 *buf = smem + cg.M / 2;
     const int tid = threadIdx.x;
@@ -1053,7 +1346,7 @@
 __global__ void __launch_bounds__(kFftThreads)
 fwd_axis1_ci_kernel(ColGeom cg, const float2 *__restrict__ tw, const float2 *__restrict__ T, float2 *__restrict__ S)
 {
-    extern __shared__ float2 smem[];
+    extern __shared__ __align__(16) float2 smem[];
     float2 *ltw = smem;
     float2 *buf = smem + cg.M / 2;
     const int tid = threadIdx.x;
@@ -1147,13 +1440,41 @@
     while ((1 << cg.logNC) < nc) ++cg.logNC;
     cg.param = g.rolloff ? 1.047197551196597746f * (float)g.m / ((float)g.N * (float)g.N) : 0.0f;
     cg.TG = nc >= 16 ? 1 : 16 / nc;
+    cg.RR = 1;
+    cg.GROUPED = 0;
+    cg.WIDE = 0;
     return cg;
 }
 
-static inline unsigned col_tiles(const ColGeom &cg, int columns = 0)
+static inline unsigned col_groups(const ColGeom &cg, int columns = 0)
 {
     const int t = ((columns > 0 ? columns : cg.KC) + cg.NC - 1) / cg.NC;
-    return (unsigned)((t + cg.TG - 1) / cg.TG * cg.TG);
+    return (unsigned)((t + cg.TG - 1) / cg.TG);
+}
+
+#ifndef NFFT_COL_MIN_WORKGROUPS
+#define NFFT_COL_MIN_WORKGROUPS 4096
+#endif
+constexpr int64_t kColMinWorkgroups = NFFT_COL_MIN_WORKGROUPS;
+constexpr int kColMaxRows = 8;
+#ifndef NFFT_COL_MODES
+#define NFFT_COL_MODES 0xa900
+#endif
+enum { kColPaired = 0, kColPlain = 1, kColGrouped = 2 };
+static dim3 col_grid(ColGeom &cg, int pass, unsigned groups, int rows, int64_t planes)
+{
+    const int mode = (NFFT_COL_MODES >> (4 * pass)) & 7;
+    cg.WIDE = (NFFT_COL_MODES >> (4 * pass + 3)) & 1;
+    cg.GROUPED = mode == kColGrouped;
+    if (!cg.GROUPED) {
+        const unsigned tiles = groups * cg.TG;
+        if (mode == kColPlain) cg.TG = 1;
+        return dim3(tiles, (unsigned)rows, (unsigned)planes);
+    }
+    int rr = 1;
+    while (rr < kColMaxRows && (int64_t)groups * ((rows + 2 * rr - 1) / (2 * rr)) * planes >= kColMinWorkgroups) rr *= 2;
+    cg.RR = rr;
+    return dim3(groups, (unsigned)((rows + rr - 1) / rr), (unsigned)planes);
 }
 
 size_t col_lds_bytes(const ColGeom &cg, bool two_buffers)
@@ -1201,8 +1522,8 @@
         if (!compact) { set_error("2-D column passes need the compact half spectrum of the own row passes"); return 4; }
         T = spec;
     } else {
-        const ColGeom cg = make_col_geom(g, false, compact);
-        const dim3 grid(col_tiles(cg), g.M, (unsigned)nplanes);
+        ColGeom cg = make_col_geom(g, false, compact);
+        const dim3 grid = col_grid(cg, 0, col_groups(cg), g.M, nplanes);
         const size_t lds = col_lds_bytes(cg, false);
         col_dispatch(cg, [&](auto lm, auto ln) {
             constexpr int LM = decltype(lm)::value, LN = decltype(ln)::value;
@@ -1214,8 +1535,8 @@
         const bool two = x_is_complex != 0;
         const int ppc = two ? 2 : 1;
         const int64_t col0 = plane0 / ppc, ncols = nplanes / ppc;
-        const ColGeom cg = make_col_geom(g, two, compact, ncols);
-        const dim3 grid(col_tiles(cg), cg.NBm, (unsigned)ncols);
+        ColGeom cg = make_col_geom(g, two, compact, ncols);
+        const dim3 grid = col_grid(cg, 1, col_groups(cg), cg.NBm, ncols);
         const size_t lds = col_lds_bytes(cg, two);
         col_dispatch(cg, [&](auto lm, auto ln) {
             constexpr int LM = decltype(lm)::value, LN = decltype(ln)::value;
@@ -1248,13 +1569,13 @@
         if (!compact) { set_error("2-D column passes need the compact half spectrum of the own row passes"); return 4; }
         T = spec;
     }
-    const ColGeom cg = make_col_geom(g, false, compact, nplanes);
+    ColGeom cg = make_col_geom(g, false, compact, nplanes);
     const size_t lds = col_lds_bytes(cg, false);
     const int ppc = real_output ? 1 : 2;
     col_dispatch(cg, [&](auto lm, auto ln) {
         constexpr int LM = decltype(lm)::value, LN = decltype(ln)::value;
         {
-            const dim3 grid(col_tiles(cg), cg.NBm, (unsigned)nplanes);
+            const dim3 grid = col_grid(cg, 2, col_groups(cg), cg.NBm, nplanes);
             if (x_is_complex) {
                 allow_lds(fwd_axis0_kernel<LM, LN, true>, lds);
                 hipLaunchKernelGGL((fwd_axis0_kernel<LM, LN, true>), grid, dim3(kFftThreads), lds, stream, cg, tw, xhat, C, ppc, plane0, T);
@@ -1264,7 +1585,7 @@
             }
         }
         if (g.dim != 2) {
-            const dim3 grid(col_tiles(cg, compact ? cg.KC : cg.Mh), g.M, (unsigned)nplanes);
+            const dim3 grid = col_grid(cg, 3, col_groups(cg, compact ? cg.KC : cg.Mh), g.M, nplanes);
             allow_lds(fwd_axis1_kernel<LM, LN>, lds);
             hipLaunchKernelGGL((fwd_axis1_kernel<LM, LN>), grid, dim3(kFftThreads), lds, stream, cg, tw, T, spec);
         }
```

Result: no change. 2776 (median of 2 runs) (-0.5%).
